# MyNiuuu/MOFA-Video

Hardware: AMD Instinct MI355X
Metric: denoised frames/sec, 25f 576x1024 SVD+MOFA, 25 steps (higher is better)
Workload: dtype f16; 1 GPU; MOFA-Video-Traj, 25-frame 576x1024, 25 denoise steps + temporal VAE decode (chunk 8), single trajectory hint, SVD-XT UNet + MOFA-Adapter, CFG 1->3, seeded random weights in the reference checkpoint layout; num_frames=25, height=576, width=1024, num_inference_steps=25, decode_chunk_size=8, parallelism=1 GPU, graph_steps=False, output_finite=True

## Files before the change

include/mofa_hip.h:

```cpp
#ifndef MOFA_HIP_H
#define MOFA_HIP_H

#include <stdint.h>

#ifdef __cplusplus
extern "C" {
#endif

typedef void* mofa_stream_t;

#define MOFA_OK 0
#define MOFA_EINVAL (-22)
#define MOFA_ELAUNCH (-5)

int mofa_version(void);

enum { MOFA_MODE_PLAIN = 0, MOFA_MODE_CONV3X3 = 1, MOFA_MODE_CONVT3 = 2 };
enum { MOFA_ACT_NONE = 0, MOFA_ACT_SILU = 1, MOFA_ACT_GEGLU_PAIR = 2, MOFA_ACT_RELU = 3,
       MOFA_ACT_GELU = 4  };

typedef struct mofa_igemm_args {
    const void* x;
    const void* w;
    const float* bias;
    const float* rowvec;
    const void* r1;
    const void* r2;
    void* out;
    int32_t M, N, Cin;
    int32_t ldx, ldo, ldr1, ldr2;
    int32_t mode;
    int32_t Hin, Win, Hout, Wout, stride, up, ksize;
    int32_t T, HW;
    int32_t rv_div, rv_mul, rv_mod_in, rv_mod_out;
    int32_t act;
    float s_acc, s1, s2;
    int32_t dil;
    int32_t pad;
    int32_t tile;
    void* workspace;
    int64_t workspace_bytes;
    float* stats;
} mofa_igemm_args;
enum { MOFA_PAD_SAME = 0, MOFA_PAD_TRAILING = 1 };
enum { MOFA_TILE_AUTO = 0, MOFA_TILE_128X128 = 2, MOFA_TILE_192X128 = 4, MOFA_TILE_256X256 = 5, MOFA_TILE_256X320 = 6 };

int mofa_igemm_f16(const mofa_igemm_args* a, mofa_stream_t stream);
int mofa_igemm_stats_ok(const mofa_igemm_args* a);
typedef struct mofa_igemm_plan_t {
    int32_t rc;
    int32_t tile, kind;
    int32_t tiles_m, tiles_n, grid, threads, lds_bytes;
    int32_t split;
    int32_t full_tiles, rem_tiles;
    int32_t stats;
    int32_t launches;
    int32_t reserved[4];
} mofa_igemm_plan_t;
int mofa_igemm_plan(const mofa_igemm_args* a, int n_cu, mofa_igemm_plan_t* out);

int mofa_attn_spatial_f16(const void* q, const void* k, const void* v, void* out,
                          int nframes, int heads, int head_dim, int S, int ldq, int ldk, int ldv, int ldo, float scale,
                          mofa_stream_t stream);
int mofa_attn_spatial_qb_f16(const void* q, const void* k, const void* v, void* out,
                             int nframes, int heads, int head_dim, int S, int ldq, int ldk, int ldv, int ldo, float scale,
                             int query_blocks, mofa_stream_t stream);
int mofa_transpose_v_f16(const void* v, void* vt, int nframes, int ncb, int S, int ldv, mofa_stream_t stream);
int mofa_attn_temporal_f16(const void* q, const void* k, const void* v, void* out,
                           int nclips, int Tq, int T, int HW, int heads, int head_dim, int ld, int ldkv, int ldo,
                           float scale, mofa_stream_t stream);
int mofa_attn_temporal_masked_f16(const void* q, const void* k, const void* v, void* out,
                                  int nclips, int Tq, int T, int HW, int heads, int head_dim, int ld, int ldkv, int ldo,
                                  float scale, uint32_t key_mask, mofa_stream_t stream);
int mofa_attn_temporal_long_f16(const void* q, const void* k, const void* v, void* out,
                                int nclips, int T, int HW, int heads, int head_dim, int ld, int ldkv, int ldo,
                                float scale, mofa_stream_t stream);
int mofa_attn_temporal_long_masked_f16(const void* q, const void* k, const void* v, void* out,
                                       int nclips, int Tq, int T, int HW, int heads, int head_dim, int ld, int ldkv, int ldo,
                                       float scale, const uint32_t* key_mask, mofa_stream_t stream);
int mofa_attn_temporal_long_local_f16(const void* q, const void* k, const void* v, void* out,
                                      int nclips, int T, int HW, int heads, int head_dim, int ld, int ldkv, int ldo,
                                      float scale, int radius, int anchor, mofa_stream_t stream);
int mofa_attn_temporal_stream_local_f16(const void* q, const void* k, const void* v, void* out,
                                        int nclips, int T, int HW, int heads, int head_dim, int ld, int ldkv, int ldo,
                                        float scale, int radius, int anchor, mofa_stream_t stream);
int mofa_softmax_rows_f16(void* x, int rows, int cols, int ld, mofa_stream_t stream);

int mofa_gn_nparts(int HW, int C);
int mofa_gn_partial_f16(const void* x, float* part, int nframes, int HW, int C, int ldx, mofa_stream_t stream);
int mofa_gn_partial_from_stats(const float* stats, float* part, int nframes, int HW, int C, mofa_stream_t stream);
int mofa_gn_finalize(const float* part, const float* gamma, const float* beta, float* scale, float* shift,
                     int nframes, int HW, int C, int frames_per_stat, float eps, mofa_stream_t stream);
int mofa_gn_reduce(const float* part, double* sums, int nframes, int HW, int C, int frames_per_stat, mofa_stream_t stream);
int mofa_gn_finalize_sums(const double* sums, const float* gamma, const float* beta, float* scale, float* shift,
                          int nframes, int C, int frames_per_stat, double count_per_group, float eps,
                          mofa_stream_t stream);
int mofa_gn_apply_f16(const void* x, const float* part, const float* gamma, const float* beta, void* y,
                      int nframes, int HW, int C, int ldx, int ldy, int frames_per_stat, float eps, int silu,
                      mofa_stream_t stream);
int mofa_gn_apply_gathered_f16(const void* x, const float* part_all, int nentries, double count_per_group,
                               const float* gamma, const float* beta, void* y, int nframes, int HW, int C,
                               int ldx, int ldy, float eps, int silu, mofa_stream_t stream);
int mofa_affine_act_f16(const void* x, const float* scale, const float* shift, void* y,
                        int nframes, int HW, int C, int ldx, int ldy, int silu, mofa_stream_t stream);
int mofa_layernorm_f16(const void* x, const float* gamma, const float* beta, void* y, int M, int C,
                       int ldx, int ldy, float eps, const float* rowvec, int rv_div, int rv_mod,
                       mofa_stream_t stream);

typedef struct mofa_ff320_args {
    const void* x;
    const float* pos;
    const void* w1p;
    const float* b1;
    const void* w2p;
    const float* b2;
    const void* r2;
    void* out;
    void* out_ln;
    const float* ln_gamma;
    const float* ln_beta;
    int32_t M, ldx, ldo, ldr2, ldoln, HW, T;
    float eps, s_acc, s1, s2, ln_eps;
    int32_t reserved[4];
} mofa_ff320_args;
int mofa_ff320_f16(const mofa_ff320_args* a, mofa_stream_t stream);

typedef struct mofa_lin320_args {
    const void* x;
    const void* wp;
    const float* bias;
    const float* rowvec;
    const void* r1;
    void* out;
    int32_t M, N, ldx, ldo, ldr1, norm;
    int32_t rv_div, rv_mul, rv_mod_in, rv_mod_out;
    float eps, s_acc, s1;
    int32_t reserved[3];
} mofa_lin320_args;
int mofa_lin320_f16(const mofa_lin320_args* a, mofa_stream_t stream);

int mofa_axpby_f32(const float* x, float* y, int64_t n, float a, float b, mofa_stream_t stream);
int mofa_resize_nearest_f32(const float* x, float* y, int n, int H, int W, int h, int w, mofa_stream_t stream);
int mofa_mask_blend_f16(const void* a, const void* b, const float* w, void* out, int M, int C, int HW, int lda,
                        int ldb, int ldo, mofa_stream_t stream);
int mofa_matting_blend_f16(const void* warped, const void* matting, const void* logit, void* out, float* mask_out,
                           int M, int C, int ldw, int ldm, int ldl, int ldo, mofa_stream_t stream);
int mofa_subsample_tokens_f16(const void* x, void* y, int n, int H, int W, int s, int C, int ldx, int ldy,
                              mofa_stream_t stream);
int mofa_axpby_f16(const void* x, void* y, int M, int C, int ldx, int ldy, float a, float b, mofa_stream_t stream);
int mofa_axpby_out_f16(const void* x, const void* y, void* out, int M, int C, int ldx, int ldy, int ldo, float a, float b,
                       mofa_stream_t stream);
int mofa_geglu_f16(const void* x, void* out, int M, int Ch, int ldx, int ldo, mofa_stream_t stream);
int mofa_copy2d_f16(const void* src, void* dst, int M, int C, int lds, int ldd, mofa_stream_t stream);
int mofa_silu_f32(const float* x, float* y, int n, mofa_stream_t stream);
int mofa_cast_f32_to_f16(const float* x, void* y, int64_t n, mofa_stream_t stream);
int mofa_cast_f16_to_f32(const void* x, float* y, int64_t n, mofa_stream_t stream);
int mofa_nchw_f32_to_nhwc_f16(const float* x, void* y, int n, int C, int HW, int ldo, float scale,
                              mofa_stream_t stream);
int mofa_nhwc_f16_to_nchw_f32(const void* x, float* y, int n, int C, int HW, int ldx, mofa_stream_t stream);
int mofa_timestep_embedding(const float* t, float* out, int n, int dim, mofa_stream_t stream);

int64_t mofa_softsplat_ws_bytes(int nflows, int H, int W);
int mofa_softsplat_avg_f16(const void* feat, const float* flow, void* out, void* ws,
                           int nflows, int H, int W, int C, int ldf, int ldo, mofa_stream_t stream);
int mofa_softsplat_scatter_f32(const float* in, const float* flow, float* out_sum, int N, int C, int H, int W,
                               mofa_stream_t stream);
int mofa_softsplat_weight_f32(const float* in, const float* metric, float* out, int N, int C, int H, int W, int mode,
                              mofa_stream_t stream);
int mofa_softsplat_normalize_f32(const float* summed, float* out, int N, int C, int H, int W, int eps_mode, mofa_stream_t stream);
typedef struct mofa_softsplat_grad_args {
    const float* grad;
    const float* flow;
    const float* in;
    const float* metric;
    const float* inv;
    const float* glast;
    float* grad_in;
    float* grad_flow;
    float* grad_metric;
    float* partial;
    int32_t N, C, H, W, prep, slices;
    int32_t reserved[4];
} mofa_softsplat_grad_args;
int mofa_softsplat_norm_f32(const float* flow, float* norm, void* ws, int N, int H, int W, mofa_stream_t stream);
int mofa_softsplat_grad_prologue_f32(const float* grad, const float* out, const float* norm, float* inv, float* glast,
                                     int N, int C, int H, int W, int eps_mode, mofa_stream_t stream);
int mofa_softsplat_grad_f32(const mofa_softsplat_grad_args* a, mofa_stream_t stream);
typedef struct mofa_softsplat_gather_args {
    const float* in;
    const float* flow;
    const float* metric;
    float* out;
    float* norm;
    void* ws;
    int32_t N, C, H, W, prep, normalize, eps_mode, slices;
    int32_t reserved[4];
} mofa_softsplat_gather_args;
int mofa_softsplat_gather_f32(const mofa_softsplat_gather_args* a, mofa_stream_t stream);
int mofa_flow_downscale_f32(const float* flow, float* out, int n, int H, int W, int s, mofa_stream_t stream);

int mofa_prepare_model_input(const float* latents, const float* image_latents, void* out,
                             int T, int HW, int ldo, float sigma, mofa_stream_t stream);
int mofa_cfg_euler_step(float* latents, const void* noise_pred, int T, int HW, int ldn,
                        float sigma, float sigma_next, float gmin, float gmax, mofa_stream_t stream);
#define MOFA_STEP_SCALARS 8
int mofa_prepare_model_input_dev(const float* latents, const float* image_latents, void* out,
                                 int T, int HW, int ldo, const float* step_scalars, mofa_stream_t stream);
int mofa_cfg_euler_step_dev(float* latents, const void* noise_pred, int T, int HW, int ldn,
                            const float* step_scalars, float gmin, float gmax, mofa_stream_t stream);
int mofa_step_select(const float* table, int* counter, float* cur, int nsteps, mofa_stream_t stream);


// ... 38 lines not shown
```

mofa_video_amd/blocks.py:

```python
import math

import torch

from . import lib as L
from . import ops
from .weights import (f32, interleave_geglu, pack_conv3d_t3, pack_conv3x3, pack_ff320, pack_lin320, pack_linear, pad_rows)

BIG = 1 << 30
LOCAL_STREAM_ABOVE = 128


class Sub:

    def __init__(self, sd, prefix="", device="cuda"):
        self.sd, self.prefix, self.device = sd, prefix, device

    def sub(self, name):
        return Sub(self.sd, f"{self.prefix}{name}.", self.device)

    def has(self, name):
        return f"{self.prefix}{name}" in self.sd

    def get(self, name):
        return self.sd[f"{self.prefix}{name}"].detach()

    def dev(self, t):
        return t.to(self.device)


class Ctx:

    def __init__(self, B, T):
        self.B, self.T = B, T
        self.N = B * T
        self.temb_act = None
        self.temb_all = None
        self.ctx16 = None
        self.cache = {}
        self.time_context_hw_major = True
        self.par = None
        self.ctx16_all = None
        self.half = 0
        self.local = None
        self.halves = None


def make_ctx(net, timestep, encoder_hidden_states, added_time_ids, B, T, base=None, half=None, par=None, local=None):
    c = base if base is not None else Ctx(B, T)
    ts = torch.as_tensor(timestep, dtype=torch.float32, device=net.device).reshape(-1)
    ts = ts.expand(B).contiguous() if ts.numel() == 1 else ts.contiguous()
    ids = added_time_ids.to(net.device, torch.float32)
    if half is not None:
        ids = ids[half:half + B]
    c.temb_act = net.time(ts, ids.contiguous())
    c.temb_all = net.temb_batch.run(c.temb_act)
    if c.ctx16 is None:
        e = encoder_hidden_states.to(net.device, torch.float32)
        e = e.reshape(e.shape[0], -1).contiguous()
        if half is not None:
            c.ctx16_all = ops.cast_f32_to_f16(e)
            c.ctx16 = c.ctx16_all[half:half + B].contiguous()
            c.half = half
        else:
            c.ctx16 = ops.cast_f32_to_f16(e)
    if local is not None and par is not None:
        raise ValueError("local temporal attention of frame-sharded clips: the gathered-key path has no per-query mask")
    c.par, c.local = par, local
    return c


class Linear:
    def __init__(self, s, pad_n=False):
        w = s.get("weight")
        w = w.reshape(w.shape[0], -1)
        self.n_real = w.shape[0]
        b = s.get("bias") if s.has("bias") else None
        if pad_n:
            w = pad_rows(w)
            b = pad_rows(b) if b is not None else None
        self.w = s.dev(pack_linear(w))
        self.b = s.dev(f32(b)) if b is not None else None

    def __call__(self, x, **kw):
        return ops.igemm(x, self.w, self.b, **kw)


class Conv3x3:
    def __init__(self, s, stride=1, up=1, pad_n=False, pad=L.PAD_SAME):
        w, b = s.get("weight"), s.get("bias")
        self.n_real = w.shape[0]
        if pad_n:
            w, b = pad_rows(w), pad_rows(b)
        self.w = s.dev(pack_conv3x3(w))
        self.b = s.dev(f32(b))
        self.stride, self.up, self.pad = stride, up, pad

    def __call__(self, x, H, W, **kw):
        return ops.igemm(x, self.w, self.b, geom=ops.conv3x3_geom(H, W, self.stride, self.up, pad=self.pad), **kw)


class ConvT3:
    def __init__(self, s, pad_n=False):
        w, b = s.get("weight"), s.get("bias")
        if pad_n:
            w, b = pad_rows(w), pad_rows(b)
        self.w = s.dev(pack_conv3d_t3(w))
        self.b = s.dev(f32(b))

    def __call__(self, x, T, HW, **kw):
        return ops.igemm(x, self.w, self.b, geom=ops.convt3_geom(T, HW), **kw)


class GroupNorm:
    def __init__(self, s, eps):
        self.g, self.b, self.eps = s.dev(f32(s.get("weight"))), s.dev(f32(s.get("bias"))), eps

    def __call__(self, x, nframes, HW, frames_per_stat=1, silu=False):
        return ops.group_norm(x, self.g, self.b, nframes, HW, self.eps, frames_per_stat, silu)


class LayerNorm:
    def __init__(self, s, eps=1e-5):
        self.g, self.b, self.eps = s.dev(f32(s.get("weight"))), s.dev(f32(s.get("bias"))), eps

    def __call__(self, x, **kw):
        return ops.layer_norm(x, self.g, self.b, self.eps, **kw)


class GegluFF:

    def __init__(self, s, norm=None, norm_eps=1e-5):
        w, b = interleave_geglu(s.get("net.0.proj.weight"), s.get("net.0.proj.bias"))
        self.w1, self.b1 = s.dev(pack_linear(w)), s.dev(f32(b))
        self.out = Linear(s.sub("net.2"))
        self.pk = None
        if norm is not None and tuple(s.get("net.0.proj.weight").shape) == (2560, 320) and tuple(s.get("net.2.weight").shape) == (320, 1280):
            w1p, b1f, w2p = pack_ff320(s.get("net.0.proj.weight"), s.get("net.0.proj.bias"), s.get("net.2.weight"),
                                       norm.get("weight"), norm.get("bias"))
            self.pk = (s.dev(w1p), s.dev(b1f), s.dev(w2p), norm_eps)

    def __call__(self, x, **epilogue):
        h = ops.igemm(x, self.w1, self.b1, act=L.ACT_GEGLU_PAIR)
        return self.out(h, **epilogue)

    @property
    def can_fuse(self):
        return self.pk is not None and ops.FF_FUSED

    def fused(self, x, **kw):
        w1p, b1f, w2p, eps = self.pk
        return ops.ff320(x, w1p, b1f, w2p, self.out.b, eps=eps, **kw)


def drive(gen):
    try:
        while True:
            next(gen)
    except StopIteration as stop:
        return stop.value


def run_lockstep(gens, enter):
    vals, live = [None] * len(gens), list(range(len(gens)))
    while live:
        for i in list(live):
            with enter[i]():
                try:
                    next(gens[i])
                except StopIteration as stop:
                    vals[i] = stop.value
                    live.remove(i)
    return vals


def _sigmoid(v):
    return 1.0 / (1.0 + math.exp(-float(v)))


class TembBatch:
    _active = None

    def __init__(self):
        self.items, self.total, self.w, self.b = [], 0, None, None

    def __enter__(self):
        self._prev, TembBatch._active = TembBatch._active, self
        return self

    def __exit__(self, *exc):
        TembBatch._active = self._prev
        if exc[0] is None and self.items:
            mult = 1
            for lin in self.items:
                mult = mult * lin.n_real // math.gcd(mult, lin.n_real)
            pad = (-self.total) % mult
            ws, bs = [lin.w for lin in self.items], [lin.b for lin in self.items]
            if pad:
                ws.append(ws[0].new_zeros((pad, ws[0].shape[1])))
                bs.append(bs[0].new_zeros((pad,)))
            self.w, self.b = torch.cat(ws, 0).contiguous(), torch.cat(bs, 0).contiguous()
            for lin in self.items:
                lin.w = lin.b = None
        return False

    def add(self, lin):
        assert lin.w.shape[0] == lin.n_real and lin.n_real % 64 == 0 and lin.b is not None
        off = self.total
        self.items.append(lin)
        self.total += lin.n_real
        return off

    def run(self, temb_act):
        return ops.cast_f16_to_f32(ops.igemm(temb_act, self.w, self.b)) if self.w is not None else None


class SpatioTemporalResBlock:

    def __init__(self, s, eps, temporal_eps=None, switch=False):
        sp, tp = s.sub("spatial_res_block"), s.sub("temporal_res_block")
        self.norm1, self.norm2 = GroupNorm(sp.sub("norm1"), eps), GroupNorm(sp.sub("norm2"), eps)
        self.conv1, self.conv2 = Conv3x3(sp.sub("conv1")), Conv3x3(sp.sub("conv2"))
        self.temb = Linear(sp.sub("time_emb_proj")) if sp.has("time_emb_proj.weight") else None
        tb = TembBatch._active
        self.temb_off = tb.add(self.temb) if (tb is not None and self.temb is not None) else None
        self.shortcut = Linear(sp.sub("conv_shortcut")) if sp.has("conv_shortcut.weight") else None
        te = temporal_eps if temporal_eps is not None else eps
        self.tnorm1, self.tnorm2 = GroupNorm(tp.sub("norm1"), te), GroupNorm(tp.sub("norm2"), te)
        self.tconv1, self.tconv2 = ConvT3(tp.sub("conv1")), ConvT3(tp.sub("conv2"))
        self.ttemb = Linear(tp.sub("time_emb_proj")) if tp.has("time_emb_proj.weight") else None
        self.ttemb_off = tb.add(self.ttemb) if (tb is not None and self.ttemb is not None) else None
        alpha = _sigmoid(s.get("time_mixer.mix_factor").reshape(-1)[0])
        self.alpha = (1.0 - alpha) if switch else alpha

    def __call__(self, x, c, H, W, out_stats=False, out=None):
        HW, N, T = H * W, c.N, c.T

        def tvec(lin, off):
            if off is not None and c.temb_all is not None:
                return dict(rowvec=c.temb_all[:, off:off + lin.n_real], rv=(T * HW, c.temb_all.shape[1] // lin.n_real, 1, BIG))
            return dict(rowvec=ops.cast_f16_to_f32(lin(c.temb_act)), rv=(T * HW, 1, 1, BIG))
        h = self.norm1(x, N, HW, silu=True)
        if self.temb is not None:
            h = self.conv1(h, H, W, stats=True, **tvec(self.temb, self.temb_off))
        else:
            h = self.conv1(h, H, W, stats=True)
        h = self.norm2(h, N, HW, silu=True)
        xs = self.shortcut(x) if self.shortcut is not None else x
        par = c.par
        xs = self.conv2(h, H, W, r1=xs, s1=1.0, stats=par is None)
        if par is None:
# ... 301 lines not shown
```

mofa_video_amd/csrc/igemm.hip:

```cpp
#include "igemm_common.h"


__device__ __forceinline__ void wait_vmcnt_le(int t) {
    if (t >= 48) wait_vmcnt<48>();
    else if (t >= 32) wait_vmcnt<32>();
    else if (t >= 24) wait_vmcnt<24>();
    else if (t >= 16) wait_vmcnt<16>();
    else if (t >= 8) wait_vmcnt<8>();
    else if (t >= 4) wait_vmcnt<4>();
    else wait_vmcnt<0>();
}

#define EPI_SLAB_BYTES 8192
__device__ __forceinline__ int slab_off(int row, int chunk) { return row * 256 + ((chunk ^ (row & 15)) << 4); }

struct PassLoads {
    f16x8 t1, t2;
    f32x4 rv0, rv1;
};

template <int EPI>
__device__ __forceinline__ void load_bias(const mofa_igemm_args& a, int ncol0, int lane, f32x4 (&b)[4]) {
    constexpr bool GEGLU = (EPI & EPI_GEGLU) != 0;
    const f32x4 z = {0, 0, 0, 0};
// ... 241 lines not shown
        for (int q = 0; q < WI; ++q) glds16(wsrc[q] + (size_t)ksw * BKS, sb + SXB + (wave * WI + q) * 1024);
        ++ksw;
        if (++ikc == kpt) { ikc = 0; ++itap; }
    };

    const int fsw = (l31 >> 1) & 7;
    const int xrow = (wm * MI * 32 + l31) * RB;
    const int wrow = SXB + (wn * NJ * 32 + l31) * RB;

    f32x4 bias[4];
    setup(walk.start + walk.local);
    {
        int lane_b = lane;
        asm volatile("" : "+v"(lane_b));
        load_bias<EPI>(a, n0 + wn * NJ * 32, lane_b, bias);
    }
    issue(0);
    int par = 0;
    int allow = 0;
    bool first = true;
    for (;;) {
        const int m0c = m0, n0c = n0;
        f32x16 acc[MI][NJ];
#pragma unroll
        for (int i = 0; i < MI; ++i)
#pragma unroll
            for (int j = 0; j < NJ; ++j)
#pragma unroll
                for (int r = 0; r < 16; ++r) acc[i][j][r] = 0.0f;
        auto compute = [&](int cur) {
            const char* sb = smem + cur * STB;
#pragma unroll
            for (int kk = 0; kk < BKS / 16; ++kk) {
                const int slot = ((kk * 2 + lh) ^ fsw) * 16;
                f16x8 xf[MI], wf[NJ];
#pragma unroll
                for (int i = 0; i < MI; ++i) xf[i] = *(const f16x8*)(sb + xrow + i * 32 * RB + slot);
#pragma unroll
                for (int j = 0; j < NJ; ++j) wf[j] = *(const f16x8*)(sb + wrow + j * 32 * RB + slot);
#pragma unroll
                for (int i = 0; i < MI; ++i)
#pragma unroll
                    for (int j = 0; j < NJ; ++j)
                        acc[i][j] = __builtin_amdgcn_mfma_f32_32x32x16_f16(wf[j], xf[i], acc[i][j], 0, 0, 0);
            }
        };
        auto compute_and_issue = [&](int cur, int nxt) {
            if (ikc == 0) {
#pragma unroll
                for (int q = 0; q < XI; ++q) xs[q] = x_src(a, geo[q], itap);
            }
            const char* sb = smem + cur * STB;
            char* nb = smem + nxt * STB;
            constexpr int OPS = XI + WI, NG = BKS / 16;
            constexpr int SPREAD = 4;
#pragma unroll
            for (int kk = 0; kk < NG; ++kk) {
#pragma unroll
                for (int o = (kk * OPS / SPREAD < OPS ? kk * OPS / SPREAD : OPS);
                     o < ((kk + 1) * OPS / SPREAD < OPS ? (kk + 1) * OPS / SPREAD : OPS); ++o) {
                    if (o < XI) {
                        const f16* sp = xs[o] ? xs[o] + ikc * BKS + xoff[o] : (const f16*)g_zero_page;
                        glds16(sp, nb + (wave * XI + o) * 1024);
                    } else {
                        glds16(wsrc[o - XI] + (size_t)ksw * BKS, nb + SXB + (wave * WI + (o - XI)) * 1024);
                    }
                }
                const int slot = ((kk * 2 + lh) ^ fsw) * 16;
                f16x8 xf[MI], wf[NJ];
#pragma unroll
                for (int i = 0; i < MI; ++i) xf[i] = *(const f16x8*)(sb + xrow + i * 32 * RB + slot);
#pragma unroll
                for (int j = 0; j < NJ; ++j) wf[j] = *(const f16x8*)(sb + wrow + j * 32 * RB + slot);
#pragma unroll
                for (int i = 0; i < MI; ++i)
#pragma unroll
                    for (int j = 0; j < NJ; ++j)
                        acc[i][j] = __builtin_amdgcn_mfma_f32_32x32x16_f16(wf[j], xf[i], acc[i][j], 0, 0, 0);
            }
            ++ksw;
            if (++ikc == kpt) { ikc = 0; ++itap; }
        };
        for (int ks = 0; ks < nk - 1; ++ks) {
            if (ks == 0) wait_vmcnt_le(allow); else wait_vmcnt<0>();
            __builtin_amdgcn_s_barrier();
            const int cur = (par + ks) & 1;
            compute_and_issue(cur, cur ^ 1);
        }
        const int last = (par + nk - 1) & 1;
        if (nk == 1) wait_vmcnt_le(allow); else wait_vmcnt<0>();
        __builtin_amdgcn_s_barrier();
        bias_touch<EPI>(bias);
        walk.local += walk.stride;
        const bool has_next = walk.local < walk.count;
        if (has_next) {
            setup(walk.start + walk.local);
            issue(last ^ 1);
        } else {
#pragma unroll
            for (int q = 0; q < XI + WI; ++q)
                glds16((const f16*)g_zero_page, smem + (last ^ 1) * STB + (wave * (XI + WI) + q) * 1024);
        }
        asm volatile("" ::: "memory");
        compute(last);
        wait_lds();
        __builtin_amdgcn_s_barrier();
        char* slab = smem + last * STB + wave * EPI_SLAB_BYTES;
        int lane_e = lane;
        asm volatile("" : "+v"(lane_e));
        if (wide) igemm_epilogue<MI, EPI, true>(a, acc, m0c + wm * MI * 32, n0c + wn * NJ * 32, lane_e, slab, bias);
        else igemm_epilogue<MI, EPI, false>(a, acc, m0c + wm * MI * 32, n0c + wn * NJ * 32, lane_e, slab, bias);
        first = false;
        if (!has_next) break;
        {
            int lane_b = lane;
            asm volatile("" : "+v"(lane_b));
            load_bias<EPI>(a, n0 + wn * NJ * 32, lane_b, bias);
        }
        allow = (wide && m0c + TBM <= a.M && n0c + TBN <= a.N) ? epi_ops + (a.bias ? (GEGLU ? 4 : 2) : 0) : 0;
        par = last ^ 1;
    }
    wait_vmcnt<0>();
}

extern "C" int mofa_igemm_f16(const mofa_igemm_args* a, mofa_stream_t stream) {
    int rc = igemm_check_args(a);
    if (rc != MOFA_OK) return rc;
#define IGEMM_KINDS(WM, WN, MI)                                                                                        \
    {igemm_f16_kernel<WM, WN, MI, 0>, igemm_f16_kernel<WM, WN, MI, 1>, igemm_f16_kernel<WM, WN, MI, 2>,                \
     igemm_f16_kernel<WM, WN, MI, 3>, igemm_f16_kernel<WM, WN, MI, 4>, igemm_f16_kernel<WM, WN, MI, 5>,                \
     igemm_f16_kernel<WM, WN, MI, 6>, igemm_f16_kernel<WM, WN, MI, 7>, igemm_f16_kernel<WM, WN, MI, 8>}
    static const igemm_kern_t k128[9] = IGEMM_KINDS(2, 2, 2), k192[9] = IGEMM_KINDS(2, 2, 3);
    static LaunchSetup setup;
    const int n_cu = setup.cus([](int) {
        return mofa_lds_optin(k128, igemm_tile(MOFA_TILE_128X128).lds) == MOFA_OK &&
                       mofa_lds_optin(k192, igemm_tile(MOFA_TILE_192X128).lds) == MOFA_OK && igemm8_init() == MOFA_OK &&
                       igemm320_init() == MOFA_OK
                   ? MOFA_OK
                   : MOFA_ELAUNCH;
    });
    if (n_cu == 0) return MOFA_ELAUNCH;
    const IgemmPlan plan = igemm_plan_checked(a, n_cu);
    if (plan.rc != MOFA_OK) return plan.rc;
    if (plan.tile == MOFA_TILE_256X320) return igemm320_launch(a, plan, (hipStream_t)stream);
    if (plan.tile == MOFA_TILE_256X256) return igemm8_launch(a, plan, (hipStream_t)stream);
    hipLaunchKernelGGL((plan.tile == MOFA_TILE_128X128 ? k128 : k192)[plan.kind], dim3(plan.grid), dim3(plan.threads), plan.lds_bytes,
                       (hipStream_t)stream, *a, plan.tiles_n, plan.full_tiles);
    MOFA_CHECK_LAUNCH();
    return MOFA_OK;
}

extern "C" int mofa_igemm_stats_ok(const mofa_igemm_args* a) { return igemm320_stats_ok(a) ? 1 : 0; }

extern "C" int mofa_igemm_plan(const mofa_igemm_args* a, int n_cu, mofa_igemm_plan_t* out) {
    if (!a || !out || n_cu <= 0) return MOFA_EINVAL;
    *out = igemm_plan(a, n_cu);
    return MOFA_OK;
}
```

mofa_video_amd/csrc/igemm320.hip:

```cpp
#include "igemm_common.h"
#include "igemm_pipe.h"

namespace {

constexpr int WN3 = 2, MI3 = 2;
constexpr int TBM3 = 256;
constexpr int RBH = 64;
constexpr int XPL = TBM3 * RBH;
constexpr int NJ3 = 5;
constexpr int TBN3 = WN3 * NJ3 * 32;
constexpr int PLANE = (TBM3 + TBN3) * RBH;
constexpr int SLOT = 2 * PLANE;
constexpr int BIAS0 = 2 * SLOT;
constexpr int LDS_BYTES3 = BIAS0 + 8 * 2 * 768;
constexpr int LOOKAHEAD3 = 4 + NJ3;

struct ScratchRows { __device__ __forceinline__ int operator()(int r) const { return (r >> 3) * 8192 + (r & 7) * 128; } };

__device__ __forceinline__ int slot_swz(int q) { return q ^ ((q & 1) << 1); }

struct Cursor3 {
    int local;
    int ikc, ksw, ky, kx;
    int gx0, gx1;
    unsigned xo0, xo1;
    int phase;
    int kend;
    unsigned wo0;
};

template <int EPI, bool SPLIT = false, bool STATS = false>
__global__ __launch_bounds__(512, 2) void igemm320_f16_kernel(const mofa_igemm_args a, const int tilesN, const int ntiles,
                                                              const Aux aux) {
    constexpr bool R1 = (EPI & EPI_R1) != 0, R2 = (EPI & EPI_R2) != 0, RV = (EPI & EPI_RV) != 0, GEGLU = (EPI & EPI_GEGLU) != 0;
    extern __shared__ __attribute__((aligned(16))) char smem[];
    TileWalk walk;
    walk.init(ntiles);
    const bool has_item = SPLIT && (int)blockIdx.x < aux.nitems;
    if (walk.local >= walk.count && !has_item) return;
    const int tid = threadIdx.x, lane = tid & 63;
    const int wave = __builtin_amdgcn_readfirstlane(tid >> 6);
    const int grp = wave >> 2;
    const int wm = wave / WN3, wn = wave - wm * WN3;
    const int l31 = lane & 31, lh = lane >> 5;

    const int taps = igemm_taps(a);
    const int kpt = a.Cin / 64, nk = taps * kpt;
    const size_t Ktot = (size_t)taps * a.Cin;

    auto swz_bytes = [&](int l, int p) __attribute__((always_inline)) { return (((l & 3) ^ slot_swz((l >> 4) & 3)) * 16 + p * RBH); };
    const TapGeo tg(a);
    const unsigned wd1 = 128u * (unsigned)(Ktot * 2), wd2 = (unsigned)(256 + 16 * (wave & 3) - 16 * wave) * (unsigned)(Ktot * 2);
    constexpr unsigned W_DEAD = 0x80000000u;
    const BufRsrc rsx = buf_rsrc(aux.xbase, aux.x_bytes), rsw = buf_rsrc(a.w, aux.w_bytes);
    const LdsDma16 bglds16;
    auto item_decode = [&](int phase, int local, int& tile, int& kb, int& ke) __attribute__((always_inline)) {
        tile = walk.start + (phase == 0 ? local : 0); kb = 0; ke = nk;
        if constexpr (SPLIT) {
            const int q = fdiv((int)blockIdx.x, aux.nsplit_d), ks = (int)blockIdx.x - q * aux.nsplit;
            const int kb1 = fdiv(ks * nk, aux.nsplit_d), ke1 = fdiv((ks + 1) * nk, aux.nsplit_d);
            const bool it = phase == 1;
            tile = it ? aux.tile0 + q : tile;
            kb = it ? kb1 : 0;
            ke = it ? ke1 : nk;
        }
    };
    auto next_pos = [&](int& phase, int& local) __attribute__((always_inline)) {
        if (phase == 0) {
            local += walk.stride;
            if (local >= walk.count) phase = has_item ? 1 : 2;
        } else {
            phase = 2;
        }
    };
    auto cur_setup = [&](Cursor3& c, const int p) __attribute__((always_inline)) {
        const bool live = c.phase < 2;
        int tile, kb, ke;
        item_decode(c.phase, c.local, tile, kb, ke);
        const int tm = fdiv(tile, aux.tiles_n), tn = tile - tm * tilesN;
        const int l = lane_now(lane), r_l = l >> 2;
        const int g0 = pack_geo(a, aux, tm * TBM3 + 16 * wave + r_l), g1 = pack_geo(a, aux, tm * TBM3 + 16 * (wave + 8) + r_l);
        c.gx0 = live ? g0 : -1;
        c.gx1 = live ? g1 : -1;
        const unsigned wo = (unsigned)(tn * TBN3 + 16 * wave + r_l) * (unsigned)(Ktot * 2) + swz_bytes(l, p);
        c.wo0 = live ? wo : W_DEAD;
        c.ikc = 0; c.ksw = 0; c.ky = 0; c.kx = 0;
        c.kend = ke;
        if constexpr (SPLIT) {
            int tap = fdiv(kb, aux.kpt_d);
            c.ikc = kb - tap * kpt;
            c.ksw = kb;
            if (a.mode == MOFA_MODE_CONV3X3) { c.ky = fdiv(tap, aux.ks_d); c.kx = tap - c.ky * tg.ks; } else c.ky = tap;
            c.xo0 = tap_src(a, aux, tg, c.gx0, c.ky, c.kx, swz_bytes(l, p));
            c.xo1 = tap_src(a, aux, tg, c.gx1, c.ky, c.kx, swz_bytes(l, p));
        }
    };
    auto issue = [&](Cursor3& c, const int p, const int slot) __attribute__((always_inline)) {
        if (c.ikc == 0) {
            const int l = lane_now(lane);
            c.xo0 = tap_src(a, aux, tg, c.gx0, c.ky, c.kx, swz_bytes(l, p));
            c.xo1 = tap_src(a, aux, tg, c.gx1, c.ky, c.kx, swz_bytes(l, p));
        }
        char* pl = smem + slot + p * PLANE;
        const int wk = c.ksw * 128;
        bglds16(rsx, c.xo0, c.ikc * 128, pl + wave * 1024);
        bglds16(rsx, c.xo1, c.ikc * 128, pl + (wave + 8) * 1024);
        bglds16(rsw, c.wo0, wk, pl + XPL + wave * 1024);
        bglds16(rsw, c.wo0 + wd1, wk, pl + XPL + (wave + 8) * 1024);
        if (grp == p) bglds16(rsw, c.wo0 + wd2, wk, pl + XPL + (16 + (wave & 3)) * 1024);
    };
    auto advance = [&](Cursor3& c, const int p) __attribute__((always_inline)) {
        tap_advance(c, a, kpt, tg.ks);
        if (c.ksw == c.kend) { next_pos(c.phase, c.local); cur_setup(c, p); }
    };

    int xa, wa;
    {
        const int r = lane & 15, c = lane >> 4;
        const int rw = 8 * ((r >> 2) & 1) + 4 * (r >> 3) + (r & 3);
        xa = (wm * MI3 * 32 + r) * RBH + (c ^ slot_swz((r >> 2) & 3)) * 16;
        wa = XPL + (wn * NJ3 * 32 + rw) * RBH + (c ^ slot_swz((rw >> 2) & 3)) * 16;
    }

    const BufRsrc rsb = buf_rsrc(a.bias, a.bias ? (unsigned)a.N * 4u : 0u);
    char* bias_lds = smem + BIAS0 + wave * 1536;
    auto bias_prefetch = [&](int phase_, int local_, int slot) __attribute__((always_inline)) {
        if (phase_ != 0) return;
        int tile_, kb_, ke_;
        item_decode(phase_, local_, tile_, kb_, ke_);
        const int tm_ = fdiv(tile_, aux.tiles_n), tn_ = tile_ - tm_ * tilesN;
        const unsigned n0 = (unsigned)(tn_ * TBN3 + wn * NJ3 * 32 + lane_now(lane));
#pragma unroll
        for (int k = 0; k < 3; ++k)
            __builtin_amdgcn_raw_ptr_buffer_load_lds(rsb, (__attribute__((address_space(3))) void*)(bias_lds + slot * 768 + k * 256), 4,
                                                     (n0 + 64u * k) * 4u, 0, 0, 0);
    };

    Cursor3 ca, cb;
    ca.local = cb.local = walk.local;
    ca.phase = cb.phase = walk.local < walk.count ? 0 : 1;
    cur_setup(ca, 0);
    cur_setup(cb, 1);
    bias_prefetch(walk.local < walk.count ? 0 : 1, walk.local, 0);
    issue(ca, 0, 0); advance(ca, 0);
    issue(cb, 1, 0); advance(cb, 1);
    issue(ca, 0, SLOT); advance(ca, 0);
    wait_vmcnt_only<LOOKAHEAD3>();
    __builtin_amdgcn_s_barrier();

    f32x16 acc[MI3][NJ3];
    f16x8 xf[2 * MI3], wf[2 * NJ3];
    auto phase = [&](auto pc, const int bo, const int bn) __attribute__((always_inline)) {
        constexpr int P = decltype(pc)::v;
#pragma unroll
        for (int i = 0; i < 2 * MI3; ++i) xf[i] = *(const f16x8*)(smem + xa + P * PLANE + i * 16 * RBH);
#pragma unroll
        for (int j = 0; j < 2 * NJ3; ++j) wf[j] = *(const f16x8*)(smem + wa + P * PLANE + j * 16 * RBH);
        __builtin_amdgcn_sched_barrier(0);
        if constexpr (P == 0) { issue(cb, 1, bn); advance(cb, 1); }
        else { issue(ca, 0, bo); advance(ca, 0); }
        wait_vmcnt<LOOKAHEAD3>();
        __builtin_amdgcn_sched_barrier(0);
        __builtin_amdgcn_s_barrier();
        __builtin_amdgcn_sched_barrier(0);
        __builtin_amdgcn_s_setprio(1);
#pragma unroll
        for (int i = 0; i < MI3; ++i)
#pragma unroll
            for (int j = 0; j < NJ3; ++j)
#pragma unroll
                for (int q = 0; q < 4; ++q) {
                    f32x4 c = {acc[i][j][4 * q], acc[i][j][4 * q + 1], acc[i][j][4 * q + 2], acc[i][j][4 * q + 3]};
                    c = __builtin_amdgcn_mfma_f32_16x16x32_f16(wf[2 * j + (q >> 1)], xf[2 * i + (q & 1)], c, 0, 0, 0);
#pragma unroll
                    for (int e = 0; e < 4; ++e) acc[i][j][4 * q + e] = c[e];
                }
        __builtin_amdgcn_s_setprio(0);
        __builtin_amdgcn_sched_barrier(0);
        __builtin_amdgcn_s_barrier();
        __builtin_amdgcn_sched_barrier(0);
    };

    auto to_layout32 = [&](f32x16 (&acc)[MI3][NJ3]) __attribute__((always_inline)) {
#pragma unroll
        for (int i = 0; i < MI3; ++i)
#pragma unroll
            for (int j = 0; j < NJ3; ++j)
#pragma unroll
                for (int v = 0; v < 2; ++v)
#pragma unroll
                    for (int s = 0; s < 4; ++s) {
                        const float lo = acc[i][j][8 * v + s], hi = acc[i][j][8 * v + 4 + s];
                        const auto sw = __builtin_amdgcn_permlane16_swap(__builtin_bit_cast(unsigned, lo), __builtin_bit_cast(unsigned, hi), false, false);
                        const unsigned slo = sw[0], shi = sw[1];
                        acc[i][j][8 * v + s] = __builtin_bit_cast(float, slo);
                        acc[i][j][8 * v + 4 + s] = __builtin_bit_cast(float, shi);
                    }
    };

    auto pin_tuples = [&](f32x16 (&acc)[MI3][NJ3]) __attribute__((always_inline)) {
#pragma unroll
        for (int i = 0; i < MI3; ++i)
#pragma unroll
            for (int j = 0; j < NJ3; ++j) asm volatile("" : "+v"(acc[i][j]));
    };

    const ScratchRows srow;
    auto epilogue_light = [&](auto ac, auto wnc, f32x16 (&acc)[MI3][NJ3], const int mw, const int nw, char* eb) __attribute__((always_inline)) {
        constexpr int J0 = decltype(wnc)::v ? 1 : 0;
        constexpr int JS = decltype(wnc)::v ? 0 : 4;
        const int lane_e = lane_now(lane);
        const int lane = lane_e, l31 = lane & 31, lh = lane >> 5;
        f16* out = (f16*)a.out;
        float saccv = a.s_acc;
        asm volatile("" : "+v"(saccv));
        char* wr = eb + srow(l31);
#pragma unroll
        for (int i = 0; i < MI3; ++i) {
#pragma unroll
            for (int pr = 0; pr < 2; ++pr) {
                const int j0 = J0 + 2 * pr;
#pragma unroll
                for (int jj = 0; jj < 2; ++jj)
#pragma unroll
                    for (int g = 0; g < 4; ++g) {
                        f16x4 o;
#pragma unroll
                        for (int e = 0; e < 4; ++e) o[e] = (f16)act_apply(ac, saccv * acc[i][j0 + jj][4 * g + e]);
                        const int c8 = 8 * jj + 2 * g + lh;
                        *(f16x4*)h16_off(wr, l31, c8) = o;
                    }
#pragma unroll
                for (int p = 0; p < 4; ++p) {
                    const H16Piece r = h16_row<8>(eb, srow, lane, p);
                    const int mr = mw + 32 * i + r.row, n = nw + 32 * j0 + 8 * r.blk;
                    if (mr < a.M && n + 8 <= a.N) *(f16x8*)(out + (size_t)mr * a.ldo + n) = r.v;
                }
            }
            {
#pragma unroll
                for (int g = 0; g < 4; ++g) {
                    f16x4 o;
#pragma unroll
                    for (int e = 0; e < 4; ++e) o[e] = (f16)act_apply(ac, saccv * acc[i][JS][4 * g + e]);
                    const int c8 = 2 * g + lh;
                    *(f16x4*)h16_off(wr, l31, c8) = o;
                }
#pragma unroll
                for (int p = 0; p < 2; ++p) {
                    const H16Piece r = h16_row<4>(eb, srow, lane, p);
                    const int mr = mw + 32 * i + r.row, n = nw + 32 * JS + 8 * r.blk;
                    if (mr < a.M && n + 8 <= a.N) *(f16x8*)(out + (size_t)mr * a.ldo + n) = r.v;
                }
            }
        }
        wait_lds();
    };
    auto epilogue_res16 = [&](auto wnc, auto unit, f32x16 (&acc)[MI3][NJ3], const int mw, const int nw, char* eb) __attribute__((always_inline)) {
        constexpr int J0 = decltype(wnc)::v ? 1 : 0;
        constexpr int JS = decltype(wnc)::v ? 0 : 4;
        constexpr bool UNIT = decltype(unit)::v != 0;
        constexpr int PPI = 10, NP = MI3 * PPI;
        const int lane_e = lane_now(lane);
        const int lane = lane_e, l31 = lane & 31, lh = lane >> 5;
        f16* out = (f16*)a.out;
        const f16* r1 = (const f16*)a.r1;
        const f16* r2 = (const f16*)a.r2;
        float s1v = a.s1, s2v = a.s2, saccv = a.s_acc;
        asm volatile("" : "+v"(s1v), "+v"(s2v), "+v"(saccv));
        auto piece_pos = [&](int st, int& mr, int& n) __attribute__((always_inline)) {
            const int i = st / PPI, q = st % PPI;
            if (q < 8) {
                mr = mw + 32 * i + 8 * (q & 3) + (lane >> 3);
                n = nw + 32 * (J0 + 2 * (q >> 2)) + 8 * (lane & 7);
            } else {
                mr = mw + 32 * i + 16 * (q - 8) + (lane >> 2);
                n = nw + 32 * JS + 8 * (lane & 3);
            }
        };
        constexpr int D = (R1 && R2) ? 2 : 5;
        f16x8 L1[D], L2[D];
        auto piece_loads = [&](int st, int slot) __attribute__((always_inline)) {
            int mr, n;
            piece_pos(st, mr, n);
            mr = mr < a.M ? mr : a.M - 1;
            n = n + 8 <= a.N ? n : 0;
            if (R1) L1[slot] = *(const f16x8*)(r1 + (size_t)mr * a.ldr1 + n);
            if (R2) L2[slot] = *(const f16x8*)(r2 + (size_t)mr * a.ldr2 + n);
        };
#pragma unroll
        for (int st = 0; st < D; ++st) piece_loads(st, st);
        auto finish = [&](int st, f16x8 o) __attribute__((always_inline)) {
            int mr, n;
            piece_pos(st, mr, n);
            if constexpr (UNIT) {
                o = o + L1[st % D];
            } else {
#pragma unroll
                for (int e = 0; e < 8; ++e) {
                    float x = (float)o[e];
                    if (R1) x += s1v * (float)L1[st % D][e];
                    if (R2) x += s2v * (float)L2[st % D][e];
                    o[e] = (f16)x;
                }
            }
            if (mr < a.M && n + 8 <= a.N) *(f16x8*)(out + (size_t)mr * a.ldo + n) = o;
            if (st + D < NP) piece_loads(st + D, st % D);
        };
        char* wr = eb + srow(l31);
#pragma unroll
        for (int i = 0; i < MI3; ++i) {
#pragma unroll
            for (int pr = 0; pr < 2; ++pr) {
                const int j0 = J0 + 2 * pr;
#pragma unroll
                for (int jj = 0; jj < 2; ++jj)
#pragma unroll
                    for (int g = 0; g < 4; ++g) {
                        f16x4 o;
#pragma unroll
                        for (int e = 0; e < 4; ++e) o[e] = (f16)(saccv * acc[i][j0 + jj][4 * g + e]);
                        const int c8 = 8 * jj + 2 * g + lh;
                        *(f16x4*)h16_off(wr, l31, c8) = o;
                    }
#pragma unroll
                for (int p = 0; p < 4; ++p) {
                    const H16Piece r = h16_row<8>(eb, srow, lane, p);
                    finish(i * PPI + pr * 4 + p, r.v);
                }
            }
            {
#pragma unroll
                for (int g = 0; g < 4; ++g) {
                    f16x4 o;
#pragma unroll
                    for (int e = 0; e < 4; ++e) o[e] = (f16)(saccv * acc[i][JS][4 * g + e]);
                    const int c8 = 2 * g + lh;
                    *(f16x4*)h16_off(wr, l31, c8) = o;
                }
#pragma unroll
                for (int p = 0; p < 2; ++p) {
                    const H16Piece r = h16_row<4>(eb, srow, lane, p);
                    finish(i * PPI + 8 + p, r.v);
                }
            }
        }
        wait_lds();
    };
    auto epilogue_stats = [&](auto wnc, f32x16 (&acc)[MI3][NJ3], const int mw, const int nw, char* eb) __attribute__((always_inline)) {
        constexpr int J0 = decltype(wnc)::v ? 1 : 0, JS = decltype(wnc)::v ? 0 : 4;
        constexpr int NP = 20;
        const int lane_e = lane_now(lane);
        const int lane = lane_e, l31 = lane & 31, lh = lane >> 5;
        f16* out = (f16*)a.out;
        const f16* r1 = (const f16*)a.r1;
        float saccv = a.s_acc;
        asm volatile("" : "+v"(saccv));
        auto piece_pos = [&](int st, int& mr, int& n) __attribute__((always_inline)) {
            if (st < 16) {
                mr = mw + 32 * ((st >> 2) & 1) + 8 * (st & 3) + (lane >> 3);
                n = nw + 32 * (J0 + 2 * (st >> 3)) + 8 * (lane & 7);
            } else {
                mr = mw + 32 * ((st - 16) >> 1) + 16 * ((st - 16) & 1) + (lane >> 2);
                n = nw + 32 * JS + 8 * (lane & 3);
            }
        };
        constexpr int D = 5;
        f16x8 L1[D];
        auto piece_loads = [&](int st, int slot) __attribute__((always_inline)) {
            int mr, n;
            piece_pos(st, mr, n);
            mr = mr < a.M ? mr : a.M - 1;
            L1[slot] = *(const f16x8*)(r1 + (size_t)mr * a.ldr1 + n);
        };
        if constexpr (R1) {
#pragma unroll
            for (int st = 0; st < D; ++st) piece_loads(st, st);
        }
        float S[4], Q[4];
        const f16x2 one2 = {(f16)1.0f, (f16)1.0f};
        auto finish = [&](int st, f16x8 o) __attribute__((always_inline)) {
            int mr, n;
            piece_pos(st, mr, n);
            if constexpr (R1) o = o + L1[st % D];
            if (mr < a.M) *(f16x8*)(out + (size_t)mr * a.ldo + n) = o;
#pragma unroll
            for (int k = 0; k < 4; ++k) {
                const f16x2 h = {o[2 * k], o[2 * k + 1]};
                S[k] = __builtin_amdgcn_fdot2(h, one2, S[k], false);
                Q[k] = __builtin_amdgcn_fdot2(h, h, Q[k], false);
            }
            asm volatile("" : "+v"(S[0]), "+v"(S[1]), "+v"(S[2]), "+v"(S[3]), "+v"(Q[0]), "+v"(Q[1]), "+v"(Q[2]), "+v"(Q[3]));
            if constexpr (R1) {
                if (st + D < NP) piece_loads(st + D, st % D);
            }
        };
        auto reduce_store = [&](const int from, const int n0, const bool writer) __attribute__((always_inline)) {
#pragma unroll
            for (int o = from; o < 64; o <<= 1) {
                const int src = (lane ^ o) << 2;
#pragma unroll
                for (int k = 0; k < 4; ++k) {
                    S[k] += __builtin_bit_cast(float, __builtin_amdgcn_ds_bpermute(src, __builtin_bit_cast(int, S[k])));
                    Q[k] += __builtin_bit_cast(float, __builtin_amdgcn_ds_bpermute(src, __builtin_bit_cast(int, Q[k])));
                }
// ... 133 lines not shown
                }
            }
        };
#pragma unroll
        for (int st = 0; st < D; ++st) step_loads(st, L[st]);
        char* wr = eb + srow(l31);
        const int wsw = ((l31 >> 1) & 3) | ((l31 & 1) << 2);
#pragma unroll
        for (int st = 0; st < STEPS; ++st) {
            const int i = st / NJ3, j = st % NJ3;
            StepLoads& l = L[st % D];
#pragma unroll
            for (int g = 0; g < 4; ++g) {
                f32x4 v;
#pragma unroll
                for (int e = 0; e < 4; ++e) v[e] = acc[i][j][4 * g + e];
                *(f32x4*)(wr + (((2 * g + lh) ^ wsw) << 4)) = v;
            }
            const int n = nw + 32 * j + 8 * piece;
#pragma unroll
            for (int p = 0; p < 2; ++p) {
                const int row = 16 * p + rrow;
                const int rsw = ((row >> 1) & 3) | ((row & 1) << 2);
                const f32x4 v0 = *(const f32x4*)(eb + srow(row) + (((2 * piece) ^ rsw) << 4));
                const f32x4 v1 = *(const f32x4*)(eb + srow(row) + (((2 * piece + 1) ^ rsw) << 4));
                f16x8 o;
#pragma unroll
                for (int e = 0; e < 4; ++e) {
                    float x0 = v0[e], x1 = v1[e];
                    if (RVROW) { x0 += l.rv0[p][e]; x1 += l.rv1[p][e]; }
                    x0 *= saccv; x1 *= saccv;
                    if (R1 || R2) { x0 = (float)(f16)x0; x1 = (float)(f16)x1; }
                    if (R1) { x0 += s1v * (float)l.t1[p][e]; x1 += s1v * (float)l.t1[p][4 + e]; }
                    if (R2) { x0 += s2v * (float)l.t2[p][e]; x1 += s2v * (float)l.t2[p][4 + e]; }
                    o[e] = (f16)x0; o[4 + e] = (f16)x1;
                }
                const int m = mw + 32 * i + row;
                if (m < a.M && n + 8 <= a.N) *(f16x8*)(out + (size_t)m * a.ldo + n) = o;
            }
            if (st + D < STEPS) step_loads(st + D, L[st % D]);
        }
        wait_lds();
    };

    auto epilogue_dump = [&](f32x16 (&acc)[MI3][NJ3], float* wst, char* eb) __attribute__((always_inline)) {
        const int lane_e = lane_now(lane);
        const int lane = lane_e, l31 = lane & 31, lh = lane >> 5;
        const int piece = lane & 3, rrow = lane >> 2;
        char* wr = eb + srow(l31);
        const int wsw = ((l31 >> 1) & 3) | ((l31 & 1) << 2);
#pragma unroll
        for (int st = 0; st < MI3 * NJ3; ++st) {
            const int i = st / NJ3, j = st % NJ3;
#pragma unroll
            for (int g = 0; g < 4; ++g) {
                f32x4 v;
#pragma unroll
                for (int e = 0; e < 4; ++e) v[e] = acc[i][j][4 * g + e];
                *(f32x4*)(wr + (((2 * g + lh) ^ wsw) << 4)) = v;
            }
#pragma unroll
            for (int p = 0; p < 2; ++p) {
                const int row = 16 * p + rrow;
                const int rsw = ((row >> 1) & 3) | ((row & 1) << 2);
                const f32x4 v0 = *(const f32x4*)(eb + srow(row) + (((2 * piece) ^ rsw) << 4));
                const f32x4 v1 = *(const f32x4*)(eb + srow(row) + (((2 * piece + 1) ^ rsw) << 4));
                float* d = wst + (size_t)(wm * MI3 * 32 + 32 * i + row) * TBN3 + wn * NJ3 * 32 + 32 * j + 8 * piece;
                *(f32x4*)d = v0;
                *(f32x4*)(d + 4) = v1;
            }
        }
        wait_lds();
    };

    int gt = 0;
    int cph = walk.local < walk.count ? 0 : 1, cl = walk.local, bslot = 0;
    for (; cph < 2; next_pos(cph, cl), bslot ^= 1) {
        int tile, kb, ke;
        item_decode(cph, cl, tile, kb, ke);
        {
            int nph = cph, nl = cl;
            next_pos(nph, nl);
            bias_prefetch(nph, nl, bslot ^ 1);
        }
        const int tm = fdiv(tile, aux.tiles_n), tn = tile - tm * tilesN;
        const int mw = tm * TBM3 + wm * MI3 * 32;
        const int nw = tn * TBN3 + wn * NJ3 * 32;
        int idx_u = -1;
        if constexpr (RV) idx_u = rowvec_uniform_idx<32 * MI3>(a, mw);
        if (SPLIT && cph == 1) {
#pragma unroll
            for (int i = 0; i < MI3; ++i)
#pragma unroll
                for (int j = 0; j < NJ3; ++j)
#pragma unroll
                    for (int r = 0; r < 16; ++r) acc[i][j][r] = 0.0f;
        } else {
            const int lane_e = lane_now(lane);
            const int col_e = 8 * ((lane_e >> 4) & 1) + 4 * (lane_e >> 5);
#pragma unroll
            for (int j = 0; j < NJ3; ++j)
#pragma unroll
                for (int v = 0; v < 2; ++v) {
                    f32x4 b = *(const f32x4*)(bias_lds + bslot * 768 + (32 * j + 16 * v + col_e) * 4);
                    if (RV && idx_u >= 0) {
                        int n = nw + 32 * j + 16 * v + col_e;
                        n = n + 4 <= a.N ? n : 0;
                        b += *(const f32x4*)(a.rowvec + (size_t)idx_u * a.N + n);
                    }
#pragma unroll
                    for (int e = 0; e < 4; ++e) {
                        acc[0][j][8 * v + e] = b[e]; acc[0][j][8 * v + 4 + e] = b[e];
                        acc[1][j][8 * v + e] = b[e]; acc[1][j][8 * v + 4 + e] = b[e];
                    }
                }
        }
        pin_tuples(acc);
        if (grp == 1) __builtin_amdgcn_s_barrier();
        for (int kt = kb; kt < ke; ++kt, ++gt) {
            const int bo = (gt & 1) * SLOT, bn = SLOT - bo;
            phase(IC<0>{}, bo, bn);
            phase(IC<1>{}, bo, bn);
            const int d = (gt & 1) ? -SLOT : SLOT;
            xa += d;
            wa += d;
        }
        if (grp == 0) __builtin_amdgcn_s_barrier();
        pin_tuples(acc);
        to_layout32(acc);
        pin_tuples(acc);

        char* eb = smem + ((gt - 1) & 1) * SLOT + PLANE + wave * 1024;
        if (SPLIT && cph == 1) {
            epilogue_dump(acc, aux.ws + (size_t)blockIdx.x * (TBM3 * TBN3), eb);
        } else if constexpr (STATS) {
            if (wn == 0) epilogue_stats(IC<0>{}, acc, mw, nw, eb);
            else epilogue_stats(IC<1>{}, acc, mw, nw, eb);
        } else if constexpr (GEGLU) {
            if (a.s_acc == 1.0f) epilogue_geglu(IC<1>{}, acc, mw, nw, eb);
            else epilogue_geglu(IC<0>{}, acc, mw, nw, eb);
        } else if constexpr (R1 || R2) {
            if (RV && idx_u < 0) {
                epilogue_rows(IC<0>{}, acc, mw, nw, eb);
            } else {
                const bool unit = R1 && !R2 && a.s1 == 1.0f;
                if (wn == 0) {
                    if (unit) epilogue_res16(IC<0>{}, IC<1>{}, acc, mw, nw, eb);
                    else epilogue_res16(IC<0>{}, IC<0>{}, acc, mw, nw, eb);
                } else {
                    if (unit) epilogue_res16(IC<1>{}, IC<1>{}, acc, mw, nw, eb);
                    else epilogue_res16(IC<1>{}, IC<0>{}, acc, mw, nw, eb);
                }
            }
        } else if (RV && idx_u < 0) {
            epilogue_rows(IC<0>{}, acc, mw, nw, eb);
        } else if (wn == 0) {
            if (RV || a.act == MOFA_ACT_NONE) epilogue_light(IC<MOFA_ACT_NONE>{}, IC<0>{}, acc, mw, nw, eb);
            else if (a.act == MOFA_ACT_SILU) epilogue_light(IC<MOFA_ACT_SILU>{}, IC<0>{}, acc, mw, nw, eb);
            else if (a.act == MOFA_ACT_RELU) epilogue_light(IC<MOFA_ACT_RELU>{}, IC<0>{}, acc, mw, nw, eb);
            else epilogue_light(IC<MOFA_ACT_GELU>{}, IC<0>{}, acc, mw, nw, eb);
        } else {
            if (RV || a.act == MOFA_ACT_NONE) epilogue_light(IC<MOFA_ACT_NONE>{}, IC<1>{}, acc, mw, nw, eb);
            else if (a.act == MOFA_ACT_SILU) epilogue_light(IC<MOFA_ACT_SILU>{}, IC<1>{}, acc, mw, nw, eb);
            else if (a.act == MOFA_ACT_RELU) epilogue_light(IC<MOFA_ACT_RELU>{}, IC<1>{}, acc, mw, nw, eb);
            else epilogue_light(IC<MOFA_ACT_GELU>{}, IC<1>{}, acc, mw, nw, eb);
        }
    }
    wait_vmcnt_only<0>();
}

typedef void (*igemm320_kern_t)(const mofa_igemm_args, const int, const int, const Aux);

__global__ __launch_bounds__(256) void igemm320_fixup_kernel(const mofa_igemm_args a, const float* __restrict__ ws, const int tile0,
                                                             const int nsplit, const int tilesN, const int R) {
    constexpr int PPR = TBN3 / 8, PPT = TBM3 * PPR;
    const long long total = (long long)R * PPT;
    for (long long idx = (long long)blockIdx.x * 256 + threadIdx.x; idx < total; idx += (long long)gridDim.x * 256) {
        const int r = (int)(idx / PPT), rem = (int)(idx - (long long)r * PPT);
        const int rr = rem / PPR, pc = rem - rr * PPR;
        const int tile = tile0 + r, tm = tile / tilesN, tn = tile - tm * tilesN;
        const int m = tm * TBM3 + rr, n = tn * TBN3 + pc * 8;
        if (m >= a.M || n + 8 > a.N) continue;
        float v[8];
#pragma unroll
        for (int e = 0; e < 8; ++e) v[e] = 0.f;
        for (int sl = 0; sl < nsplit; ++sl) {
            const float* q = ws + ((size_t)(r * nsplit + sl) * TBM3 + rr) * TBN3 + pc * 8;
            const f32x4 p0 = *(const f32x4*)q, p1 = *(const f32x4*)(q + 4);
#pragma unroll
            for (int e = 0; e < 4; ++e) { v[e] += p0[e]; v[4 + e] += p1[e]; }
        }
        if (a.bias) {
#pragma unroll
            for (int e = 0; e < 8; ++e) v[e] += a.bias[n + e];
        }
        if (a.rowvec) {
            const int idx_rv = ((m / a.rv_div) * a.rv_mul + (m % a.rv_mod_in)) % a.rv_mod_out;
            const float* q = a.rowvec + (size_t)idx_rv * a.N + n;
#pragma unroll
            for (int e = 0; e < 8; ++e) v[e] += q[e];
        }
#pragma unroll
        for (int e = 0; e < 8; ++e) v[e] *= a.s_acc;
        if (a.r1 || a.r2) {
#pragma unroll
            for (int e = 0; e < 8; ++e) v[e] = (float)(f16)v[e];
        }
        if (a.r1) {
            const f16x8 t = *(const f16x8*)((const f16*)a.r1 + (size_t)m * a.ldr1 + n);
#pragma unroll
            for (int e = 0; e < 8; ++e) v[e] += a.s1 * (float)t[e];
        }
        if (a.r2) {
            const f16x8 t = *(const f16x8*)((const f16*)a.r2 + (size_t)m * a.ldr2 + n);
#pragma unroll
            for (int e = 0; e < 8; ++e) v[e] += a.s2 * (float)t[e];
        }
        f16x8 o;
#pragma unroll
        for (int e = 0; e < 8; ++e) {
            float x = v[e];
            if (a.act == MOFA_ACT_SILU) x = silu_f(x);
            else if (a.act == MOFA_ACT_RELU) x = fmaxf(x, 0.0f);
            else if (a.act == MOFA_ACT_GELU) x = gelu_erf_f(x);
            o[e] = (f16)x;
        }
        *(f16x8*)((f16*)a.out + (size_t)m * a.ldo + n) = o;
    }
}

__global__ __launch_bounds__(192) void igemm320_tile_stats_kernel(const f16* __restrict__ out, const int ldo, float* __restrict__ stats,
                                                                  const int M, const int N, const int tile0, const int tilesN) {
    const int tile = tile0 + (int)(blockIdx.x >> 2), tm = tile / tilesN, tn = tile - tm * tilesN;
    const int m0 = tm * TBM3 + 64 * (int)(blockIdx.x & 3), n = tn * TBN3 + 2 * (int)threadIdx.x;
    if (m0 >= M || (int)threadIdx.x >= TBN3 / 2 || n + 2 > N) return;
    const f16x2 one2 = {(f16)1.0f, (f16)1.0f};
    float sm = 0.f, q = 0.f;
    const f16* p = out + (size_t)m0 * ldo + n;
#pragma unroll 8
    for (int r = 0; r < 64; ++r) {
        const f16x2 h = *(const f16x2*)(p + (size_t)r * ldo);
        sm = __builtin_amdgcn_fdot2(h, one2, sm, false);
        q = __builtin_amdgcn_fdot2(h, h, q, false);
    }
    float* sp = stats + (size_t)(m0 >> 6) * N + n;
    sp[0] = sm;
    sp[1] = q;
}

}

static const igemm320_kern_t k_igemm320[9] = {igemm320_f16_kernel<0>, igemm320_f16_kernel<1>, igemm320_f16_kernel<2>,
                                               igemm320_f16_kernel<3>, igemm320_f16_kernel<4>, igemm320_f16_kernel<5>,
                                               igemm320_f16_kernel<6>, nullptr, igemm320_f16_kernel<8>};
static const igemm320_kern_t k_igemm320_split[7] = {
    igemm320_f16_kernel<0, true>, igemm320_f16_kernel<1, true>, igemm320_f16_kernel<2, true>, igemm320_f16_kernel<3, true>,
    igemm320_f16_kernel<4, true>, igemm320_f16_kernel<5, true>, igemm320_f16_kernel<6, true>};

static const igemm320_kern_t k_igemm320_stats[7] = {igemm320_f16_kernel<0, false, true>, igemm320_f16_kernel<1, false, true>, nullptr,
                                                     nullptr, igemm320_f16_kernel<4, false, true>, igemm320_f16_kernel<5, false, true>, nullptr};
static const igemm320_kern_t k_igemm320_split_stats[7] = {igemm320_f16_kernel<0, true, true>, igemm320_f16_kernel<1, true, true>, nullptr,
                                                           nullptr, igemm320_f16_kernel<4, true, true>, igemm320_f16_kernel<5, true, true>, nullptr};

int igemm320_init() {
    return mofa_lds_optin(k_igemm320, LDS_BYTES3) == MOFA_OK && mofa_lds_optin(k_igemm320_split, LDS_BYTES3) == MOFA_OK &&
                   mofa_lds_optin(k_igemm320_stats, LDS_BYTES3) == MOFA_OK && mofa_lds_optin(k_igemm320_split_stats, LDS_BYTES3) == MOFA_OK
               ? MOFA_OK
               : MOFA_ELAUNCH;
}

static_assert(TBM3 == 256 && TBN3 == 320 && LDS_BYTES3 == 159744, "igemm_plan.h's MOFA_TILE_256X320 row");
int igemm320_launch(const mofa_igemm_args* a, const IgemmPlan& plan, hipStream_t stream) {
    const int kind = plan.kind, S = plan.split, R = plan.rem_tiles, tilesN = plan.tiles_n;
    Aux aux = igemm_pipe_aux(a, igemm_taps(*a), tilesN);
    igemm320_kern_t kern = a->stats ? k_igemm320_stats[kind] : k_igemm320[kind];
    if (S > 1) {
        kern = a->stats ? k_igemm320_split_stats[kind] : k_igemm320_split[kind];
        aux.nsplit = S, aux.nsplit_d = fastdiv_make(S);
        aux.tile0 = plan.full_tiles, aux.nitems = R * S, aux.ws = (float*)a->workspace;
    }
    hipLaunchKernelGGL(kern, dim3(plan.grid), dim3(plan.threads), plan.lds_bytes, stream, *a, tilesN, plan.full_tiles, aux);
    MOFA_CHECK_LAUNCH();
    if (S == 1) return MOFA_OK;
    const long long pieces = (long long)R * TBM3 * (TBN3 / 8);
    hipLaunchKernelGGL(igemm320_fixup_kernel, dim3((int)((pieces + 255) / 256)), dim3(256), 0, stream, *a,
                       (const float*)a->workspace, plan.full_tiles, S, tilesN, R);
    MOFA_CHECK_LAUNCH();
    if (a->stats) {
        hipLaunchKernelGGL(igemm320_tile_stats_kernel, dim3(R * 4), dim3(192), 0, stream, (const f16*)a->out, a->ldo, a->stats, a->M,
                           a->N, plan.full_tiles, tilesN);
        MOFA_CHECK_LAUNCH();
    }
    return MOFA_OK;
}
```

mofa_video_amd/csrc/igemm8.hip:

```cpp
#include "igemm_common.h"
#include "igemm_pipe.h"

namespace {

constexpr int WM = 2, WN = 4, MI = 4, NJ = 2;
constexpr int TBM = WM * MI * 32, TBN = WN * NJ * 32;
constexpr int BKS = 64, RB = 128;
constexpr int SXB = TBM * RB, STB = SXB + TBN * RB;
constexpr int SCRATCH0 = 2 * STB, SCRATCH_WAVE = 4096;
constexpr int LDS_BYTES = SCRATCH0 + 8 * SCRATCH_WAVE;
constexpr int LOOKAHEAD_OPS = 8;

struct Cursor {
    int local;
    int ikc, ksw, ky, kx;
    int gx0, gx1;
    unsigned xo0, xo1;
    unsigned wo0, wo1, wo2, wo3;
};

template <int EPI, int VAR = 0>
__global__ __launch_bounds__(512, 2) void igemm8_f16_kernel(const mofa_igemm_args a, const int tilesN, const int ntiles,
                                                            const Aux aux) {
    constexpr bool GEGLU = (EPI & EPI_GEGLU) != 0, R1 = (EPI & EPI_R1) != 0, R2 = (EPI & EPI_R2) != 0,
                   RV = (EPI & EPI_RV) != 0;
    extern __shared__ __attribute__((aligned(16))) char smem[];
    TileWalk walk;
    walk.init(ntiles);
    if (walk.local >= walk.count) return;
    const int tid = threadIdx.x, lane = tid & 63;
    const int wave = __builtin_amdgcn_readfirstlane(tid >> 6);
    const int grp = wave >> 2;
    const int wm = wave / WN, wn = wave - wm * WN;
    const int l31 = lane & 31, lh = lane >> 5;

    const int taps = igemm_taps(a);
    const int kpt = a.Cin / BKS, nk = taps * kpt;
    const size_t Ktot = (size_t)taps * a.Cin;

    auto swz_bytes = [&](int l, int q) __attribute__((always_inline)) { return (((l & 7) ^ (4 * q + (l >> 4))) * 16); };
    auto x_row = [&](int h, int q, int hr0) __attribute__((always_inline)) { const int hr = hr0 + 8 * q; return (hr >> 6) * 128 + h * 64 + (hr & 63); };
    auto w_row = [&](int h, int q, int hr0) __attribute__((always_inline)) { const int hr = hr0 + 8 * q; return (hr >> 5) * 64 + h * 32 + (hr & 31); };
    const TapGeo tg(a);
    const BufRsrc rsx = buf_rsrc(aux.xbase, aux.x_bytes), rsw = buf_rsrc(a.w, aux.w_bytes);
    const LdsDma16 bglds16;
    auto cur_setup = [&](Cursor& c, const int h, const bool with_w) __attribute__((always_inline)) {
        const bool live = c.local < walk.count;
        const int tile = walk.start + (live ? c.local : 0);
        const int tm = fdiv(tile, aux.tiles_n), tn = tile - tm * tilesN;
        const int l = lane_now(lane), hr_l = 16 * wave + (l >> 3);
        const int g0 = pack_geo(a, aux, tm * TBM + x_row(h, 0, hr_l)), g1 = pack_geo(a, aux, tm * TBM + x_row(h, 1, hr_l));
        c.gx0 = live ? g0 : -1;
        c.gx1 = live ? g1 : -1;
        if (with_w) {
            auto w_off = [&](int hq) __attribute__((always_inline)) {
                int n = tn * TBN + w_row(hq >> 1, hq & 1, hr_l);
                n = n < a.N ? n : a.N - 1;
                const unsigned o = (unsigned)n * (unsigned)(Ktot * 2) + swz_bytes(l, hq & 1);
                return live ? o : XO_INVALID;
            };
            c.wo0 = w_off(0); c.wo1 = w_off(1); c.wo2 = w_off(2); c.wo3 = w_off(3);
        }
        c.ikc = 0; c.ksw = 0; c.ky = 0; c.kx = 0;
    };
    auto issue_x = [&](Cursor& c, const int h, const int bo) __attribute__((always_inline)) {
        if (c.ikc == 0) {
            const int l = lane_now(lane);
            c.xo0 = tap_src(a, aux, tg, c.gx0, c.ky, c.kx, swz_bytes(l, 0));
            c.xo1 = tap_src(a, aux, tg, c.gx1, c.ky, c.kx, swz_bytes(l, 1));
        }
        bglds16(rsx, c.xo0, c.ikc * (BKS * 2), smem + bo + x_row(h, 0, 16 * wave) * RB);
        bglds16(rsx, c.xo1, c.ikc * (BKS * 2), smem + bo + x_row(h, 1, 16 * wave) * RB);
    };
    auto issue_w = [&](Cursor& c, const int bo) __attribute__((always_inline)) {
        bglds16(rsw, c.wo0, c.ksw * (BKS * 2), smem + bo + SXB + w_row(0, 0, 16 * wave) * RB);
        bglds16(rsw, c.wo1, c.ksw * (BKS * 2), smem + bo + SXB + w_row(0, 1, 16 * wave) * RB);
        bglds16(rsw, c.wo2, c.ksw * (BKS * 2), smem + bo + SXB + w_row(1, 0, 16 * wave) * RB);
        bglds16(rsw, c.wo3, c.ksw * (BKS * 2), smem + bo + SXB + w_row(1, 1, 16 * wave) * RB);
    };
    auto advance = [&](Cursor& c, const int h, const bool with_w) __attribute__((always_inline)) {
        tap_advance(c, a, kpt, tg.ks);
        if (c.ksw == nk) { c.local += walk.stride; cur_setup(c, h, with_w); }
    };

    int xa[4], wa[4];
    {
        const int fsw = (l31 >> 1) & 7;
#pragma unroll
        for (int kk = 0; kk < 4; ++kk) {
            const int slot = ((kk * 2 + lh) ^ fsw) * 16;
            xa[kk] = (wm * MI * 32 + l31) * RB + slot;
            wa[kk] = SXB + (wn * NJ * 32 + l31) * RB + slot;
        }
    }

    char* scr = smem + SCRATCH0 + wave * SCRATCH_WAVE;
    const BufRsrc rsb = buf_rsrc(a.bias, a.bias ? (unsigned)a.N * 4u : 0u);
    auto bias_prefetch = [&](int nw, int slot = 0) __attribute__((always_inline)) {
        __builtin_amdgcn_raw_ptr_buffer_load_lds(rsb, (__attribute__((address_space(3))) void*)(scr + slot * 256), 4,
                                                 (unsigned)(nw + lane_now(lane)) * 4u, 0, 0, 0);
    };
    constexpr bool BIAS_INIT = GEGLU;

    Cursor ca, cb;
    ca.local = cb.local = walk.local;
    cur_setup(ca, 0, true);
    cur_setup(cb, 1, false);
    if constexpr (BIAS_INIT) {
        const int tile0 = walk.start + walk.local;
        bias_prefetch((tile0 - fdiv(tile0, aux.tiles_n) * tilesN) * TBN + wn * NJ * 32, 0);
    }
    issue_x(ca, 0, 0); issue_w(ca, 0); advance(ca, 0, true);
    issue_x(cb, 1, 0); advance(cb, 1, false);
    issue_x(ca, 0, STB); issue_w(ca, STB); advance(ca, 0, true);
    wait_vmcnt_only<LOOKAHEAD_OPS>();
    __builtin_amdgcn_s_barrier();

    f32x16 acc[MI][NJ];
    f16x8 xf[2][4], wf[2][4];
    unsigned long long tr[13] = {0, 0, 0, 0, 0, 0, 0, 0, 0, 0, 0, 0, 0}, tr_t = 0;
    if (VAR & 64) tr_t = __builtin_readcyclecounter();
    if (VAR & 32) {
#pragma unroll
        for (int kk = 0; kk < 4; ++kk) {
            xf[0][kk] = *(const f16x8*)(smem + xa[kk]);
            xf[1][kk] = *(const f16x8*)(smem + xa[kk] + 32 * RB);
            wf[0][kk] = *(const f16x8*)(smem + wa[kk]);
            wf[1][kk] = *(const f16x8*)(smem + wa[kk] + 32 * RB);
        }
    }
    auto stamp = [&](int k) __attribute__((always_inline)) {
        if (VAR & 64) { const unsigned long long t = __builtin_readcyclecounter(); tr[k] += t - tr_t; tr_t = t; }
    };
    auto phase = [&](auto pc, const int bo, const int bn) __attribute__((always_inline)) {
        constexpr int P = decltype(pc)::v;
        auto reads = [&]() __attribute__((always_inline)) {
            if (VAR & 32) return;
#pragma unroll
            for (int il = 0; il < 2; ++il)
#pragma unroll
                for (int kk = 0; kk < 4; ++kk)
                    xf[il][kk] = *(const f16x8*)(smem + xa[kk] + ((P == 2 ? 2 : 0) + il) * 32 * RB);
            if constexpr (P == 1) {
#pragma unroll
                for (int j = 0; j < 2; ++j)
#pragma unroll
                    for (int kk = 0; kk < 4; ++kk) wf[j][kk] = *(const f16x8*)(smem + wa[kk] + j * 32 * RB);
            }
        };
        auto issues = [&]() __attribute__((always_inline)) {
            if (VAR & 16) return;
            if constexpr (P == 1) issue_x(cb, 1, bn);
            if constexpr (P == 2) { issue_x(ca, 0, bo); issue_w(ca, bo); }
        };
        if (VAR & 4) { issues(); __builtin_amdgcn_sched_barrier(0); reads(); }
        else { reads(); __builtin_amdgcn_sched_barrier(0); issues(); }
        if constexpr (P == 1) advance(cb, 1, false);
        if constexpr (P == 2) advance(ca, 0, true);
        if (!(VAR & 8)) wait_vmcnt<LOOKAHEAD_OPS>(); else wait_lds();
        __builtin_amdgcn_sched_barrier(0);
        __builtin_amdgcn_s_barrier();
        __builtin_amdgcn_sched_barrier(0);
        stamp(3 * (P - 1));
        if (!(VAR & 2)) __builtin_amdgcn_s_setprio(1);
#pragma unroll
        for (int kk = 0; kk < 4; ++kk)
#pragma unroll
            for (int il = 0; il < 2; ++il)
#pragma unroll
                for (int j = 0; j < 2; ++j) {
                    constexpr int I0 = (P == 2) ? 2 : 0;
                    acc[I0 + il][j] = __builtin_amdgcn_mfma_f32_32x32x16_f16(wf[j][kk], xf[il][kk], acc[I0 + il][j], 0, 0, 0);
                }
        if (!(VAR & 2)) __builtin_amdgcn_s_setprio(0);
        stamp(3 * (P - 1) + 1);
        __builtin_amdgcn_sched_barrier(0);
        __builtin_amdgcn_s_barrier();
        __builtin_amdgcn_sched_barrier(0);
        stamp(3 * (P - 1) + 2);
    };

    auto epilogue_light = [&](auto ac, auto un, f32x16 (&acc)[MI][NJ], const int mw, const int nw, const int idx_u) __attribute__((always_inline)) {
        constexpr bool UNI = decltype(un)::v != 0;
        constexpr bool SACC1 = GEGLU && UNI;
        const int lane_e = RV ? lane_now(lane) : lane;
        const int lane = lane_e, l31 = lane & 31, lh = lane >> 5;
        f16* out = (f16*)a.out;
        float saccv = a.s_acc;
        asm volatile("" : "+v"(saccv));
        f32x4 bv[NJ][4];
        if (!BIAS_INIT && (!RV || UNI)) {
#pragma unroll
            for (int j = 0; j < NJ; ++j)
#pragma unroll
                for (int g = 0; g < 4; ++g) bv[j][g] = *(const f32x4*)(scr + (32 * j + 8 * g + 4 * lh) * 4);
        }
        const int nout = GEGLU ? a.N / 2 : a.N;
        int rv_div = a.rv_div, rv_mod_in = a.rv_mod_in, rv_mod_out = a.rv_mod_out;
        asm volatile("" : "+s"(rv_div), "+s"(rv_mod_in), "+s"(rv_mod_out));
        f32x4 rv[NJ][4];
        auto rv_load = [&](int i, f32x4 (&rv)[NJ][4]) __attribute__((always_inline)) {
            int m = mw + 32 * i + l31;
            m = m < a.M ? m : a.M - 1;
            const int idx = UNI ? idx_u : ((m / rv_div) * a.rv_mul + (m % rv_mod_in)) % rv_mod_out;
            const float* rvp = a.rowvec + (size_t)idx * a.N;
#pragma unroll
            for (int j = 0; j < NJ; ++j)
#pragma unroll
                for (int g = 0; g < 4; ++g) {
                    int n = nw + 32 * j + 8 * g + 4 * lh;
                    n = n + 4 <= a.N ? n : 0;
                    rv[j][g] = *(const f32x4*)(rvp + n);
                    if (!UNI && a.bias) rv[j][g] += *(const f32x4*)(a.bias + n);
                }
        };
        if (RV) rv_load(0, rv);
        if (RV && UNI) {
#pragma unroll
            for (int j = 0; j < NJ; ++j)
#pragma unroll
                for (int g = 0; g < 4; ++g) bv[j][g] += rv[j][g];
        }
        auto store_pair = [&](f16x4 g0, f16x4 g1, int m, int n0) __attribute__((always_inline)) {
            typedef unsigned u32x2 __attribute__((ext_vector_type(2)));
            typedef unsigned u32x4 __attribute__((ext_vector_type(4)));
            u32x2 a2 = __builtin_bit_cast(u32x2, g0), b2 = __builtin_bit_cast(u32x2, g1);
            const auto rx = __builtin_amdgcn_permlane32_swap(a2[0], b2[0], false, false);
            const auto ry = __builtin_amdgcn_permlane32_swap(a2[1], b2[1], false, false);
            const u32x4 v = {rx[0], ry[0], rx[1], ry[1]};
            const int n = n0 + 8 * lh;
            if (m < a.M && n + 8 <= nout) *(u32x4*)(out + (size_t)m * a.ldo + n) = v;
        };
#pragma unroll
        for (int i = 0; i < MI; ++i) {
            const int m = mw + 32 * i + l31;
            if constexpr (GEGLU) {
                f16x4 o[4];
#pragma unroll
                for (int g = 0; g < 4; ++g)
#pragma unroll
                    for (int e = 0; e < 4; ++e) {
                        const float val = acc[i][g >> 1][4 * (g & 1) + e];
                        const float gate = acc[i][g >> 1][8 + 4 * (g & 1) + e];
                        if constexpr (SACC1) o[g][e] = (f16)(val * (gate * gelu_phi_f(gate)));
                        else o[g][e] = (f16)(saccv * val * gelu_erf_f(saccv * gate));
                    }
                store_pair(o[0], o[1], m, nw / 2);
                store_pair(o[2], o[3], m, nw / 2 + 16);
            } else {
#pragma unroll
                for (int j = 0; j < NJ; ++j)
#pragma unroll
                    for (int g = 0; g < 4; ++g) {
                        f16x4 o;
#pragma unroll
                        for (int e = 0; e < 4; ++e) {
                            const float v = acc[i][j][4 * g + e] + (RV && !UNI ? rv[j][g][e] : bv[j][g][e]);
                            o[e] = (f16)act_apply(ac, saccv * v);
                        }
                        *(f16x4*)(scr + h16_off(l31 * 128, l31, 8 * j + 2 * g + lh)) = o;
                    }
                if (RV && !UNI && i + 1 < MI) rv_load(i + 1, rv);
#pragma unroll
                for (int p = 0; p < 4; ++p) {
                    const H16Piece r = h16_row<4 * NJ>(scr, RowLines128{}, lane, p);
                    const int mr = mw + 32 * i + r.row, n = nw + 8 * r.blk;
                    if (mr < a.M && n + 8 <= nout) *(f16x8*)(out + (size_t)mr * a.ldo + n) = r.v;
                }
            }
        }
    };
    auto epilogue_residual = [&](auto un, f32x16 (&acc)[MI][NJ], const int mw, const int nw, const int idx_u) __attribute__((always_inline)) {
        constexpr bool UNI = decltype(un)::v != 0;
        constexpr int STEPS = MI * NJ;
        constexpr int REGS = (R1 ? 8 : 0) + (R2 ? 8 : 0) + (RV && !UNI ? 16 : 0);
        constexpr int D0 = REGS <= 8 ? 8 : (REGS <= 16 ? 4 : (REGS <= 24 ? 2 : 1));
        constexpr int D = RV && UNI ? (REGS <= 8 ? 4 : 2) : (RV ? 1 : D0);
        const int lane_e = RV ? lane_now(lane) : lane;
        const int lane = lane_e, l31 = lane & 31, lh = lane >> 5;
        f16* out = (f16*)a.out;
        const f16* r1 = (const f16*)a.r1;
        const f16* r2 = (const f16*)a.r2;
        float s1v = a.s1, s2v = a.s2, saccv = a.s_acc;
        asm volatile("" : "+v"(s1v), "+v"(s2v), "+v"(saccv));
        int rv_div = a.rv_div, rv_mod_in = a.rv_mod_in, rv_mod_out = a.rv_mod_out;
        asm volatile("" : "+s"(rv_div), "+s"(rv_mod_in), "+s"(rv_mod_out));
        const int piece = lane & 3;
        struct StepLoads { f16x8 t1[2], t2[2]; f32x4 rv0[2], rv1[2]; };
        StepLoads L[D];
        auto step_loads = [&](int st, StepLoads& l) __attribute__((always_inline)) {
            const int i = st / NJ, j = st % NJ;
            const int n = nw + 32 * j + 8 * piece;
            const int nc = n + 8 <= a.N ? n : 0;
#pragma unroll
            for (int p = 0; p < 2; ++p) {
                int m = mw + 32 * i + 16 * p + (lane >> 2);
                m = m < a.M ? m : a.M - 1;
                if (R1) l.t1[p] = *(const f16x8*)(r1 + (size_t)m * a.ldr1 + nc);
                if (R2) l.t2[p] = *(const f16x8*)(r2 + (size_t)m * a.ldr2 + nc);
                if (RV && !UNI) {
                    const int idx = ((m / rv_div) * a.rv_mul + (m % rv_mod_in)) % rv_mod_out;
                    const float* q = a.rowvec + (size_t)idx * a.N + nc;
                    l.rv0[p] = *(const f32x4*)q;
                    l.rv1[p] = *(const f32x4*)(q + 4);
                }
            }
        };
        f32x4 rvu[NJ][2];
        if (RV && UNI) {
#pragma unroll
            for (int j = 0; j < NJ; ++j) {
                const int n = nw + 32 * j + 8 * piece;
                const float* q = a.rowvec + (size_t)idx_u * a.N + (n + 8 <= a.N ? n : 0);
                rvu[j][0] = *(const f32x4*)q;
                rvu[j][1] = *(const f32x4*)(q + 4);
            }
        }
#pragma unroll
        for (int st = 0; st < D && st < STEPS; ++st) step_loads(st, L[st]);
        f32x4 bv[NJ][2];
#pragma unroll
        for (int j = 0; j < NJ; ++j) {
            bv[j][0] = *(const f32x4*)(scr + (32 * j + 8 * piece) * 4);
            bv[j][1] = *(const f32x4*)(scr + (32 * j + 8 * piece + 4) * 4);
            if (RV && UNI) { bv[j][0] += rvu[j][0]; bv[j][1] += rvu[j][1]; }
        }
#pragma unroll
        for (int st = 0; st < STEPS; ++st) {
            const int i = st / NJ, j = st % NJ;
            StepLoads& l = L[st % D];
#pragma unroll
            for (int g = 0; g < 4; ++g) {
                f32x4 v;
#pragma unroll
                for (int e = 0; e < 4; ++e) v[e] = acc[i][j][4 * g + e];
                *(f32x4*)(scr + f32_off(l31 * 128, l31, 2 * g + lh)) = v;
            }
            const int n = nw + 32 * j + 8 * piece;
#pragma unroll
            for (int p = 0; p < 2; ++p) {
                const int row = 16 * p + (lane >> 2);
                const f32x4 v0 = *(const f32x4*)(scr + f32_off(row * 128, row, 2 * piece));
                const f32x4 v1 = *(const f32x4*)(scr + f32_off(row * 128, row, 2 * piece + 1));
                f16x8 o;
#pragma unroll
                for (int e = 0; e < 4; ++e) {
                    float x0 = v0[e] + bv[j][0][e], x1 = v1[e] + bv[j][1][e];
                    if (RV && !UNI) { x0 += l.rv0[p][e]; x1 += l.rv1[p][e]; }
                    x0 *= saccv; x1 *= saccv;
                    if (R1 || R2) { x0 = (float)(f16)x0; x1 = (float)(f16)x1; }
                    if (R1) { x0 += s1v * (float)l.t1[p][e]; x1 += s1v * (float)l.t1[p][4 + e]; }
                    if (R2) { x0 += s2v * (float)l.t2[p][e]; x1 += s2v * (float)l.t2[p][4 + e]; }
                    o[e] = (f16)x0; o[4 + e] = (f16)x1;
                }
                const int m = mw + 32 * i + row;
                if (m < a.M && n + 8 <= a.N) *(f16x8*)(out + (size_t)m * a.ldo + n) = o;
            }
            if (st + D < STEPS) step_loads(st + D, L[st % D]);
        }
    };

    int gt = 0;
    int bslot = 0;
    for (int cl = walk.local; cl < walk.count; cl += walk.stride, bslot ^= 1) {
        const int tile = walk.start + cl;
        const int tm = fdiv(tile, aux.tiles_n), tn = tile - tm * tilesN;
        if (VAR & 64) { stamp(9); tr[12] += nk; }
        if constexpr (BIAS_INIT) {
            int tn2 = tn;
            if (cl + walk.stride < walk.count) {
                const int tile2 = walk.start + cl + walk.stride;
                tn2 = tile2 - fdiv(tile2, aux.tiles_n) * tilesN;
            }
            bias_prefetch(tn2 * TBN + wn * NJ * 32, bslot ^ 1);
            const int lh_e = lane_now(lane) >> 5;
#pragma unroll
            for (int j = 0; j < NJ; ++j)
#pragma unroll
                for (int g = 0; g < 4; ++g) {
                    const f32x4 b = *(const f32x4*)(scr + bslot * 256 + (32 * j + 8 * g + 4 * lh_e) * 4);
#pragma unroll
                    for (int i = 0; i < MI; ++i)
#pragma unroll
                        for (int e = 0; e < 4; ++e) acc[i][j][4 * g + e] = b[e];
                }
        } else {
#pragma unroll
            for (int i = 0; i < MI; ++i)
#pragma unroll
                for (int j = 0; j < NJ; ++j)
#pragma unroll
                    for (int r = 0; r < 16; ++r) acc[i][j][r] = 0.0f;

            bias_prefetch(tn * TBN + wn * NJ * 32);
        }
        if (!(VAR & 1) && grp == 1) __builtin_amdgcn_s_barrier();
        for (int kt = 0; kt < nk; ++kt, ++gt) {
            const int bo = (gt & 1) * STB, bn = STB - bo;
            phase(IC<1>{}, bo, bn);
            phase(IC<2>{}, bo, bn);
#pragma unroll
            for (int kk = 0; kk < 4; ++kk) { xa[kk] ^= STB; wa[kk] ^= STB; }
        }
        if (!(VAR & 1) && grp == 0) __builtin_amdgcn_s_barrier();
        stamp(6);

        const int mw = tm * TBM + wm * MI * 32;
        const int nw = tn * TBN + wn * NJ * 32;
        int idx_u = -1;
        if constexpr (RV) idx_u = rowvec_uniform_idx<32 * MI>(a, mw);
        if constexpr (R1 || R2) {
            if (RV && idx_u >= 0) epilogue_residual(IC<1>{}, acc, mw, nw, idx_u);
            else epilogue_residual(IC<0>{}, acc, mw, nw, 0);
        } else if constexpr (GEGLU) {
            if (a.s_acc == 1.0f) epilogue_light(IC<MOFA_ACT_NONE>{}, IC<1>{}, acc, mw, nw, 0);
            else epilogue_light(IC<MOFA_ACT_NONE>{}, IC<0>{}, acc, mw, nw, 0);
        } else if constexpr (RV) {
            if (idx_u >= 0) epilogue_light(IC<MOFA_ACT_NONE>{}, IC<1>{}, acc, mw, nw, idx_u);
            else epilogue_light(IC<MOFA_ACT_NONE>{}, IC<0>{}, acc, mw, nw, 0);
        } else {
            if (a.act == MOFA_ACT_NONE) epilogue_light(IC<MOFA_ACT_NONE>{}, IC<0>{}, acc, mw, nw, 0);
            else if (a.act == MOFA_ACT_SILU) epilogue_light(IC<MOFA_ACT_SILU>{}, IC<0>{}, acc, mw, nw, 0);
            else if (a.act == MOFA_ACT_RELU) epilogue_light(IC<MOFA_ACT_RELU>{}, IC<0>{}, acc, mw, nw, 0);
            else epilogue_light(IC<MOFA_ACT_GELU>{}, IC<0>{}, acc, mw, nw, 0);
        }
        if (VAR & 64) { stamp(7); tr[8] += 1; }
    }
    wait_vmcnt_only<0>();
    if ((VAR & 64) && aux.trace && (tid & 255) == 0) {
#pragma unroll
        for (int k = 0; k < 13; ++k) aux.trace[((size_t)blockIdx.x * 2 + grp) * 16 + k] = tr[k];
    }
}

typedef void (*igemm8_kern_t)(const mofa_igemm_args, const int, const int, const Aux);

}

static const igemm8_kern_t k_igemm8[9] = {igemm8_f16_kernel<0>, igemm8_f16_kernel<1>, igemm8_f16_kernel<2>,
                                           igemm8_f16_kernel<3>, igemm8_f16_kernel<4>, igemm8_f16_kernel<5>,
                                           igemm8_f16_kernel<6>, igemm8_f16_kernel<7>, igemm8_f16_kernel<8>};


#ifdef MOFA_PROBE
static int s_probe_var = 0;
static unsigned long long* s_probe_trace = nullptr;
static const int k_probe_vars[] = {1, 2, 4, 8, 16, 32, 48, 64};
static const igemm8_kern_t k_trace_kern[9] = {nullptr, igemm8_f16_kernel<1, 64>, nullptr, nullptr, igemm8_f16_kernel<4, 64>, nullptr, nullptr,
                                               nullptr, igemm8_f16_kernel<8, 64>};
static const igemm8_kern_t k_probe_kern[] = {
    igemm8_f16_kernel<0, 1>, igemm8_f16_kernel<0, 2>, igemm8_f16_kernel<0, 4>, igemm8_f16_kernel<0, 8>,
    igemm8_f16_kernel<0, 16>, igemm8_f16_kernel<0, 32>, igemm8_f16_kernel<0, 48>, igemm8_f16_kernel<0, 64>};
extern "C" int mofa_igemm8_set_probe(int var, void* trace) {
    s_probe_var = var;
    s_probe_trace = (unsigned long long*)trace;
    return 0;
}
#endif

int igemm8_init() {
    if (mofa_lds_optin(k_igemm8, LDS_BYTES) != MOFA_OK) return MOFA_ELAUNCH;
#ifdef MOFA_PROBE
    if (mofa_lds_optin(k_probe_kern, LDS_BYTES) != MOFA_OK || mofa_lds_optin(k_trace_kern, LDS_BYTES) != MOFA_OK) return MOFA_ELAUNCH;
#endif
    return MOFA_OK;
}

int igemm8_launch(const mofa_igemm_args* a, const IgemmPlan& plan, hipStream_t stream) {
    static_assert(TBM == 256 && TBN == 256 && LDS_BYTES == 163840, "igemm_plan.h's MOFA_TILE_256X256 row");
    const int kind = plan.kind;
    Aux aux = igemm_pipe_aux(a, igemm_taps(*a), plan.tiles_n);
    igemm8_kern_t kern = k_igemm8[kind];
#ifdef MOFA_PROBE
    aux.trace = s_probe_trace;
    if (kind == 0 && s_probe_var)
        for (size_t i = 0; i < sizeof(k_probe_vars) / sizeof(int); ++i)
            if (k_probe_vars[i] == s_probe_var) kern = k_probe_kern[i];
    if (s_probe_var == 64 && k_trace_kern[kind]) kern = k_trace_kern[kind];
#endif
    hipLaunchKernelGGL(kern, dim3(plan.grid), dim3(plan.threads), plan.lds_bytes, stream, *a, plan.tiles_n, plan.full_tiles, aux);
    MOFA_CHECK_LAUNCH();
    return MOFA_OK;
}
```

mofa_video_amd/csrc/igemm_pipe.h:

```cpp
#pragma once
#include "igemm_common.h"

namespace {

struct FastDiv { unsigned mul, shr; };
__device__ __forceinline__ int fdiv(int n, const FastDiv d) { return d.mul ? (int)(__umulhi((unsigned)n, d.mul) >> d.shr) : n; }

struct Aux {
    FastDiv tiles_n, hw, wout, t3hw, t3t;
    int ldxb;
    int row_shift;
    const void* xbase;
    unsigned x_bytes, w_bytes;
    unsigned long long* trace;
    FastDiv nsplit_d, kpt_d, ks_d;
    int nsplit, tile0, nitems;
    float* ws;
};

constexpr unsigned XO_INVALID = 0xffffffffu;

template <int V> struct IC { static constexpr int v = V; };

__device__ __forceinline__ int lane_now(int lane) { asm volatile("" : "+v"(lane)); return lane; }

struct TapGeo {
    int ks, dil, org;
    __device__ __forceinline__ TapGeo(const mofa_igemm_args& a)
        : ks(a.ksize > 0 ? a.ksize : 3), dil(a.dil > 0 ? a.dil : 1), org(a.pad == MOFA_PAD_TRAILING ? 0 : (ks >> 1)) {}
};

__device__ __forceinline__ int pack_geo(const mofa_igemm_args& a, const Aux& aux, int m) {
    int g = m;
    if (a.mode == MOFA_MODE_CONV3X3) {
        const int img = fdiv(m, aux.hw), rem = m - img * (a.Hout * a.Wout);
        const int oy = fdiv(rem, aux.wout);
        g = (img << 20) | (oy << 10) | (rem - oy * a.Wout);
    } else if (a.mode == MOFA_MODE_CONVT3) {
        int lo = 1, hi = 1;
        if (a.T > 0) {
            const int fr = fdiv(m, aux.t3hw);
            const int f = fr - fdiv(fr, aux.t3t) * a.T;
            lo = f > 0; hi = f < a.T - 1;
        }
        g = m | (lo << 29) | (hi << 30);
    }
    return m < a.M ? g : -1;
}

__device__ __forceinline__ unsigned tap_src(const mofa_igemm_args& a, const Aux& aux, const TapGeo& t, int g, int ky, int kx, int swzb) {
    int row = g;
    bool ok = g >= 0;
    if (a.mode == MOFA_MODE_CONV3X3) {
        const int vy = ((g >> 10) & 1023) * a.stride + (ky - t.org) * t.dil;
        const int vx = (g & 1023) * a.stride + (kx - t.org) * t.dil;
        ok = ok && vy >= 0 && vx >= 0 && vy < a.Hin * a.up && vx < a.Win * a.up;
        const int iy = (a.up == 2) ? (vy >> 1) : vy, ix = (a.up == 2) ? (vx >> 1) : vx;
        row = ((g >> 20) * a.Hin + iy) * a.Win + ix;
    } else if (a.mode == MOFA_MODE_CONVT3) {
        ok = ok && !(ky == 0 && !((g >> 29) & 1)) && !(ky == 2 && !((g >> 30) & 1));
        row = (g & 0x1fffffff) + (ky - 1) * a.HW + aux.row_shift;
    }
    const unsigned off = (unsigned)row * (unsigned)aux.ldxb + (unsigned)swzb;
    return ok ? off : XO_INVALID;
}

template <class C>
__device__ __forceinline__ void tap_advance(C& c, const mofa_igemm_args& a, const int kpt, const int ks) {
    ++c.ksw;
    if (++c.ikc == kpt) {
        c.ikc = 0;
        if (a.mode == MOFA_MODE_CONV3X3) { if (++c.kx == ks) { c.kx = 0; ++c.ky; } } else ++c.ky;
    }
}

typedef decltype(__builtin_amdgcn_make_buffer_rsrc((void*)nullptr, (short)0, 0, 0)) BufRsrc;
__device__ __forceinline__ BufRsrc buf_rsrc(const void* p, unsigned bytes) {
    return __builtin_amdgcn_make_buffer_rsrc((void*)p, 0, bytes, 0x00020000);
}
struct LdsDma16 {
    __device__ __forceinline__ void operator()(const BufRsrc& rs, unsigned voff, int soff, char* lds_wave_base) const {
        __builtin_amdgcn_raw_ptr_buffer_load_lds(rs, (__attribute__((address_space(3))) void*)lds_wave_base, 16, voff, soff, 0, 0);
    }
};

template <int ACT>
__device__ __forceinline__ float act_apply(IC<ACT>, float v) {
    if constexpr (ACT == MOFA_ACT_SILU) return silu_f(v);
    else if constexpr (ACT == MOFA_ACT_RELU) return fmaxf(v, 0.0f);
    else if constexpr (ACT == MOFA_ACT_GELU) return gelu_erf_f(v);
    else return v;
}

template <int ROWS>
__device__ __forceinline__ int rowvec_uniform_idx(const mofa_igemm_args& a, const int mw) {
    int idx_u = -1;
    if (a.rv_mod_in == 1) {
        int rv_div = a.rv_div;
        asm volatile("" : "+s"(rv_div));
        const int m0 = mw < a.M ? mw : a.M - 1, m1 = mw + ROWS - 1 < a.M ? mw + ROWS - 1 : a.M - 1;
        const int q0 = m0 / rv_div, q1 = m1 / rv_div;
        if (q0 == q1) idx_u = (q0 * a.rv_mul) % a.rv_mod_out;
    }
    return __builtin_amdgcn_readfirstlane(idx_u);
}

struct RowLines128 { __device__ __forceinline__ int operator()(int r) const { return r * 128; } };
template <class B>
__device__ __forceinline__ B h16_off(B rb, int r, int c8) {
    return rb + (((c8 >> 1) ^ ((r >> 1) & 7)) << 4) + (((c8 & 1) ^ (r & 1)) << 3);
}
__device__ __forceinline__ f16x8 h16_row_fix(int r, f16x8 v) {
    f16x8 o = v;
    if (r & 1) o = (f16x8){v[4], v[5], v[6], v[7], v[0], v[1], v[2], v[3]};
    return o;
}
template <class B>
__device__ __forceinline__ B f32_off(B rb, int r, int c) {
    return rb + ((c ^ (((r >> 1) & 3) | ((r & 1) << 2))) << 4);
}

struct H16Piece { int row, blk; f16x8 v; };
template <int CPR, class RowLines>
__device__ __forceinline__ H16Piece h16_row(const char* sb, RowLines rl, int lane, int p) {
    constexpr int SH = CPR == 8 ? 3 : (CPR == 4 ? 2 : 1);
    static_assert(CPR == 1 << SH, "8, 4 or 2 pieces per row");
    const int row = (64 >> SH) * p + (lane >> SH), blk = lane & (CPR - 1);
    const f16x8 v = *(const f16x8*)(sb + rl(row) + ((blk ^ ((row >> 1) & 7)) << 4));
    return H16Piece{row, blk, h16_row_fix(row, v)};
}

}

static inline FastDiv fastdiv_make(int d) {
    FastDiv f = {0, 0};
    if (d > 1) {
        unsigned lg = 0;
        while ((1u << lg) < (unsigned)d) ++lg;
        const unsigned p = 31 + lg;
        f.mul = (unsigned)(((1ull << p) + (unsigned)d - 1) / (unsigned)d);
        f.shr = p - 32;
    }
    return f;
}

static inline Aux igemm_pipe_aux(const mofa_igemm_args* a, int taps, int tilesN) {
    Aux aux;
    aux.tiles_n = fastdiv_make(tilesN);
    aux.hw = fastdiv_make(a->mode == MOFA_MODE_CONV3X3 ? a->Hout * a->Wout : 1);
    aux.wout = fastdiv_make(a->mode == MOFA_MODE_CONV3X3 ? a->Wout : 1);
    aux.t3hw = fastdiv_make(a->mode == MOFA_MODE_CONVT3 ? a->HW : 1);
    aux.t3t = fastdiv_make(a->mode == MOFA_MODE_CONVT3 && a->T > 0 ? a->T : 1);
    const bool halo = a->mode == MOFA_MODE_CONVT3 && a->T == 0;
    aux.ldxb = a->ldx * 2;
    aux.row_shift = halo ? a->HW : 0;
    aux.xbase = (const char*)a->x - (halo ? (size_t)a->HW * a->ldx * 2 : 0);
    aux.x_bytes = (unsigned)(igemm8_rows_in(a) * a->ldx * 2 - (a->ldx - a->Cin) * 2);
    aux.w_bytes = (unsigned)((long long)a->N * taps * a->Cin * 2);
    aux.trace = nullptr;
    aux.nsplit_d = fastdiv_make(1);
    aux.kpt_d = fastdiv_make(a->Cin / 64);
    aux.ks_d = fastdiv_make(a->mode == MOFA_MODE_CONV3X3 ? (a->ksize > 0 ? a->ksize : 3) : 1);
    aux.nsplit = 1;
    aux.tile0 = 0;
    aux.nitems = 0;
    aux.ws = nullptr;
    return aux;
}
```

mofa_video_amd/csrc/igemm_plan.h:

```cpp
#pragma once
#include <stdint.h>
#include "../../include/mofa_hip.h"

typedef mofa_igemm_plan_t IgemmPlan;

struct IgemmTile { int tm, tn, threads, lds, wg_per_cu; };
static inline const IgemmTile& igemm_tile(int id) {
    static const IgemmTile tiles[4] = {
        {128, 128, 256, 2 * 256 * 128, 2},
        {192, 128, 256, 2 * 320 * 128, 2},
        {256, 256, 512, 163840, 1},
        {256, 320, 512, 159744, 1},
    };
    return tiles[id == MOFA_TILE_128X128 ? 0 : id == MOFA_TILE_192X128 ? 1 : id == MOFA_TILE_256X256 ? 2 : 3];
}

static inline int igemm_cdiv(int64_t a, int64_t b) { return (int)((a + b - 1) / b); }

__attribute__((always_inline)) constexpr int igemm_taps(const mofa_igemm_args& a) {
    return (a.mode == MOFA_MODE_CONV3X3) ? (a.ksize > 0 ? a.ksize * a.ksize : 9) : (a.mode == MOFA_MODE_CONVT3 ? 3 : 1);
}

static inline int igemm_grid(long long ntiles, int slots) {
    const int grid = (int)(ntiles < slots ? ((ntiles + 7) / 8) * 8 : (slots / 8) * 8);
    return grid < 8 ? 8 : grid;
}

static inline long long igemm8_rows_in(const mofa_igemm_args* a) {
    if (a->mode == MOFA_MODE_CONV3X3) return a->M / ((long long)a->Hout * a->Wout) * a->Hin * a->Win;
    if (a->mode == MOFA_MODE_CONVT3 && a->T == 0) return (long long)a->M + 2ll * a->HW;
    return a->M;
}

static inline bool igemm_pipe_eligible(const mofa_igemm_args* a, int kind, long long Ktot) {
    const int nout = kind == 8 ? a->N / 2 : a->N;
    if ((a->ldo & 7) || (nout & 7) || (a->N & 7) || (((uintptr_t)a->out) & 15) || (((uintptr_t)a->x) & 15)) return false;
    if (a->r1 && ((a->ldr1 & 7) || (((uintptr_t)a->r1) & 15))) return false;
    if (a->r2 && ((a->ldr2 & 7) || (((uintptr_t)a->r2) & 15))) return false;
    if (a->bias && (((uintptr_t)a->bias) & 15)) return false;
    if ((a->r1 || a->r2 || a->rowvec) && a->act != MOFA_ACT_NONE) return false;
    if (a->rowvec && (((uintptr_t)a->rowvec) & 15)) return false;
    if ((long long)a->N * Ktot * 2 >= (1ll << 32) || (((uintptr_t)a->w) & 15)) return false;
    if (a->mode == MOFA_MODE_CONV3X3) {
        const long long nimg = a->M / ((long long)a->Hout * a->Wout);
        if (a->Hout > 1024 || a->Wout > 1024 || nimg > 2047) return false;
    } else if (a->mode == MOFA_MODE_CONVT3) {
        if (a->M >= (1 << 29)) return false;
    }
    if (igemm8_rows_in(a) * a->ldx * 2 >= (1ll << 32) - 65536) return false;
    return true;
}

static inline bool igemm320_eligible(const mofa_igemm_args* a, int kind, int taps) {
    if (kind == 7 || !igemm_pipe_eligible(a, kind, (long long)taps * a->Cin)) return false;
    return (long long)(a->N + 320) * taps * a->Cin * 2 < 0x7ff00000LL;
}

static inline bool igemm320_stats_ok(const mofa_igemm_args* a) {
    if (!a || !a->x || !a->w || !a->out || a->M <= 0 || a->N <= 0 || a->Cin <= 0 || a->Cin % 64 != 0) return false;
    if (a->act != MOFA_ACT_NONE || a->r2 || (a->r1 && a->s1 != 1.0f)) return false;
    if (a->M % 64 != 0 || a->N % 320 != 0) return false;
    if (a->rowvec && (a->rv_mod_in != 1 || a->rv_div <= 0 || a->rv_div % 64 != 0)) return false;
    if (a->tile != 0 && a->tile != MOFA_TILE_256X320) return false;
    return igemm320_eligible(a, (a->r1 ? 1 : 0) | (a->rowvec ? 4 : 0), igemm_taps(*a));
}

static inline int igemm320_split(long long T, int nk, int n_cu, long long ws_bytes) {
    const long long R = T % n_cu;
    if (ws_bytes <= 0 || R == 0) return 1;
    if (T > n_cu && R * 10 > (long long)n_cu * 6) return 1;
    long long s = n_cu / R;
    if (s > 8) s = 8;
    if (s > nk / 8) s = nk / 8;
    if (s >= 2 && 2.0 * nk * (1.0 - 1.0 / (double)s) < 50.0) s = 1;
    const long long per = (long long)256 * 320 * 4;
    while (s >= 2 && R * s * per > ws_bytes) --s;
    return s >= 2 ? (int)s : 1;
}

static inline int igemm_check_args(const mofa_igemm_args* a) {
    if (!a || !a->x || !a->w || !a->out) return MOFA_EINVAL;
    if (a->M <= 0 || a->N <= 0 || a->Cin <= 0) return MOFA_EINVAL;
    if (a->Cin % 64 != 0 || a->N % 4 != 0) return MOFA_EINVAL;
    if (a->mode < 0 || a->mode > 2 || a->act < 0 || a->act > MOFA_ACT_GELU) return MOFA_EINVAL;
    if (a->mode == MOFA_MODE_CONV3X3) {
        if (a->Hin <= 0 || a->Win <= 0 || a->Hout <= 0 || a->Wout <= 0) return MOFA_EINVAL;
        if ((a->stride != 1 && a->stride != 2) || (a->up != 1 && a->up != 2)) return MOFA_EINVAL;
        if (a->ksize != 0 && a->ksize != 1 && a->ksize != 3 && a->ksize != 5 && a->ksize != 7) return MOFA_EINVAL;
        if (a->dil < 0 || (a->dil > 1 && a->up != 1)) return MOFA_EINVAL;
        if (a->pad != MOFA_PAD_SAME && a->pad != MOFA_PAD_TRAILING) return MOFA_EINVAL;
        if (a->M % (a->Hout * a->Wout) != 0 || a->Hout > 65535 || a->Wout > 65535) return MOFA_EINVAL;
    }
    if (a->mode == MOFA_MODE_CONVT3 && (a->T < 0 || a->HW <= 0 || (a->T > 0 && a->M % (a->T * a->HW) != 0)))
        return MOFA_EINVAL;
    if (a->rowvec && (a->rv_div <= 0 || a->rv_mod_in <= 0 || a->rv_mod_out <= 0)) return MOFA_EINVAL;
    if (a->act == MOFA_ACT_GEGLU_PAIR && (a->N % 64 != 0 || a->r1 || a->r2 || a->rowvec)) return MOFA_EINVAL;
    if (a->ldx % 8 != 0 || a->ldo % 4 != 0) return MOFA_EINVAL;
    if ((a->r1 && a->ldr1 % 4 != 0) || (a->r2 && a->ldr2 % 4 != 0)) return MOFA_EINVAL;
    if (a->tile != 0 && a->tile != MOFA_TILE_128X128 && a->tile != MOFA_TILE_192X128 && a->tile != MOFA_TILE_256X256 &&
        a->tile != MOFA_TILE_256X320)
        return MOFA_EINVAL;
    if (a->stats && !igemm320_stats_ok(a)) return MOFA_EINVAL;
    return MOFA_OK;
}

static inline int igemm_model_tile(const mofa_igemm_args* a, int kind, long long Ktot, int n_cu) {
    static const double rel[2] = {1.00, 0.86};
    static const int ids[2] = {MOFA_TILE_128X128, MOFA_TILE_192X128};
    static const double epi4[9] = {2.0, 3.5, 4.0, 4.0, 3.5, 4.0, 4.5, 4.5, 4.0};
    static const double epi8[9] = {2.2, 5.2, 5.2, 6.0, 5.6, 5.5, 5.5, 6.3, 2.4};
    const double nk = (double)(Ktot / 64);
    int choice = 0;
    double best = 0;
    for (int k = 0; k < 2; ++k) {
        const IgemmTile& c = igemm_tile(ids[k]);
        const long long t = (long long)igemm_cdiv(a->M, c.tm) * igemm_cdiv(a->N, c.tn);
        const long long slots_k = (long long)n_cu * c.wg_per_cu;
        const double cost = (double)((t + slots_k - 1) / slots_k) * c.tm * c.tn * rel[k] * c.wg_per_cu * (1.0 + epi4[kind] / nk);
        if (choice == 0 || cost < best) { best = cost; choice = ids[k]; }
    }
    {
        const long long t = (long long)igemm_cdiv(a->M, 256) * igemm_cdiv(a->N, 256);
        const double cost = (double)((t + n_cu - 1) / n_cu) * 256 * 256 * 0.62 * (1.0 + epi8[kind] / nk);
        if (cost < best) { best = cost; choice = MOFA_TILE_256X256; }
    }
    if (kind != 7) {
        static const double epi320[9] = {3.0, 7.5, 8.5, 9.5, 3.5, 7.9, 9.0, 12.0, 5.0};
        const long long t = (long long)igemm_cdiv(a->M, 256) * igemm_cdiv(a->N, 320);
        const int S = kind == 8 ? 1 : igemm320_split(t, (int)nk, n_cu, a->workspace ? a->workspace_bytes : 0);
        const double rounds = S > 1 ? (double)(t / n_cu) + 1.0 / S + 0.12 : (double)((t + n_cu - 1) / n_cu);
        const int tn320 = igemm_cdiv(a->N, 320);
        const double wide = 1.0 + (tn320 > 6 ? (tn320 - 6 > 12 ? 0.25 : 0.02 * (tn320 - 6)) : 0.0);
        const double cost = rounds * 256 * 320 * 0.58 * wide * (1.0 + epi320[kind] / nk);
        if (cost < best) { best = cost; choice = MOFA_TILE_256X320; }
    }
    return choice;
}

static inline IgemmPlan igemm_plan_checked(const mofa_igemm_args* a, int n_cu) {
    IgemmPlan p = {};
    const IgemmPlan refused = {MOFA_EINVAL};
    n_cu = n_cu >= 8 ? (n_cu / 8) * 8 : 8;
    const int taps = igemm_taps(*a);
    const long long Ktot = (long long)taps * a->Cin;
    const int kind = a->act == MOFA_ACT_GEGLU_PAIR ? 8 : ((a->r1 ? 1 : 0) | (a->r2 ? 2 : 0) | (a->rowvec ? 4 : 0));
    const bool forced = a->tile != 0 || a->stats;
    int choice = a->stats ? MOFA_TILE_256X320 : a->tile != 0 ? a->tile : igemm_model_tile(a, kind, Ktot, n_cu);
    static const int chain[3] = {MOFA_TILE_256X320, MOFA_TILE_256X256, MOFA_TILE_192X128};
    for (int i = 0; i < 2; ++i) {
        if (choice != chain[i]) continue;
        if (i == 0 ? (a->stats || igemm320_eligible(a, kind, taps)) : igemm_pipe_eligible(a, kind, Ktot)) break;
        if (forced) return refused;
        choice = chain[i + 1];
    }
    const IgemmTile& c = igemm_tile(choice);
    const int tilesM = igemm_cdiv(a->M, c.tm), tilesN = igemm_cdiv(a->N, c.tn);
    const long long nt = (long long)tilesM * tilesN;
    if (nt > 0x7fffffffLL) return refused;
    if (a->stats && (((uintptr_t)a->stats) & 15)) return refused;
    const int slots = n_cu * c.wg_per_cu;
    p.tile = choice; p.kind = kind; p.tiles_m = tilesM; p.tiles_n = tilesN; p.threads = c.threads; p.lds_bytes = c.lds;
    p.grid = igemm_grid(nt, slots);
    p.split = 1; p.full_tiles = (int)nt; p.launches = 1;
    p.stats = a->stats ? 1 : 0;
    if (choice == MOFA_TILE_256X320 && kind != 8) {
        const bool ws_ok = a->workspace && (((uintptr_t)a->workspace) & 15) == 0;
        p.split = igemm320_split(nt, (int)(Ktot / 64), n_cu, ws_ok ? a->workspace_bytes : 0);
    }
    if (p.split > 1) {
        p.full_tiles = (int)(nt - nt % n_cu);
        p.rem_tiles = (int)(nt % n_cu);
        p.grid = p.full_tiles > 0 ? (n_cu / 8) * 8 : ((p.rem_tiles * p.split + 7) / 8) * 8;
        p.launches = a->stats ? 3 : 2;
        if (p.grid < p.rem_tiles * p.split) return refused;
    }
    return p;
}

static inline IgemmPlan igemm_plan(const mofa_igemm_args* a, int n_cu) {
    const IgemmPlan refused = {igemm_check_args(a)};
    return refused.rc == MOFA_OK ? igemm_plan_checked(a, n_cu) : refused;
}
```

mofa_video_amd/lib.py:

```python
import ctypes as C
import os

import torch

_HERE = os.path.dirname(os.path.abspath(__file__))
LIB_PATH = os.environ.get("MOFA_HIP_LIB") or os.path.join(_HERE, "libmofa_hip.so")

MODE_PLAIN, MODE_CONV3X3, MODE_CONVT3 = 0, 1, 2
ACT_NONE, ACT_SILU, ACT_GEGLU_PAIR, ACT_RELU, ACT_GELU = 0, 1, 2, 3, 4
PAD_SAME, PAD_TRAILING = 0, 1
SPARSE_ADD, SPARSE_LAST = 0, 1
TILE_AUTO, TILE_128X128, TILE_192X128, TILE_256X256, TILE_256X320 = 0, 2, 4, 5, 6


class IgemmArgs(C.Structure):
    _fields_ = [
        ("x", C.c_void_p), ("w", C.c_void_p), ("bias", C.c_void_p), ("rowvec", C.c_void_p),
        ("r1", C.c_void_p), ("r2", C.c_void_p), ("out", C.c_void_p),
        ("M", C.c_int32), ("N", C.c_int32), ("Cin", C.c_int32),
        ("ldx", C.c_int32), ("ldo", C.c_int32), ("ldr1", C.c_int32), ("ldr2", C.c_int32),
        ("mode", C.c_int32),
        ("Hin", C.c_int32), ("Win", C.c_int32), ("Hout", C.c_int32), ("Wout", C.c_int32),
        ("stride", C.c_int32), ("up", C.c_int32), ("ksize", C.c_int32),
        ("T", C.c_int32), ("HW", C.c_int32),
        ("rv_div", C.c_int32), ("rv_mul", C.c_int32), ("rv_mod_in", C.c_int32), ("rv_mod_out", C.c_int32),
        ("act", C.c_int32),
        ("s_acc", C.c_float), ("s1", C.c_float), ("s2", C.c_float),
        ("dil", C.c_int32), ("pad", C.c_int32), ("tile", C.c_int32),
        ("workspace", C.c_void_p), ("workspace_bytes", C.c_int64),
        ("stats", C.c_void_p),
    ]


class IgemmPlan(C.Structure):
    _fields_ = [(n, C.c_int32) for n in ("rc", "tile", "kind", "tiles_m", "tiles_n", "grid", "threads", "lds_bytes", "split",
                                         "full_tiles", "rem_tiles", "stats", "launches")] + [("reserved", C.c_int32 * 4)]


class Ff320Args(C.Structure):
    _fields_ = [
        ("x", C.c_void_p), ("pos", C.c_void_p), ("w1p", C.c_void_p), ("b1", C.c_void_p), ("w2p", C.c_void_p), ("b2", C.c_void_p),
        ("r2", C.c_void_p), ("out", C.c_void_p), ("out_ln", C.c_void_p), ("ln_gamma", C.c_void_p), ("ln_beta", C.c_void_p),
        ("M", C.c_int32), ("ldx", C.c_int32), ("ldo", C.c_int32), ("ldr2", C.c_int32), ("ldoln", C.c_int32),
        ("HW", C.c_int32), ("T", C.c_int32),
        ("eps", C.c_float), ("s_acc", C.c_float), ("s1", C.c_float), ("s2", C.c_float), ("ln_eps", C.c_float),
        ("reserved", C.c_int32 * 4),
    ]


class Lin320Args(C.Structure):
    _fields_ = [
        ("x", C.c_void_p), ("wp", C.c_void_p), ("bias", C.c_void_p), ("rowvec", C.c_void_p), ("r1", C.c_void_p), ("out", C.c_void_p),
        ("M", C.c_int32), ("N", C.c_int32), ("ldx", C.c_int32), ("ldo", C.c_int32), ("ldr1", C.c_int32), ("norm", C.c_int32),
        ("rv_div", C.c_int32), ("rv_mul", C.c_int32), ("rv_mod_in", C.c_int32), ("rv_mod_out", C.c_int32),
        ("eps", C.c_float), ("s_acc", C.c_float), ("s1", C.c_float),
        ("reserved", C.c_int32 * 3),
    ]


class SoftsplatGradArgs(C.Structure):
    _fields_ = [
        ("grad", C.c_void_p), ("flow", C.c_void_p), ("inp", C.c_void_p), ("metric", C.c_void_p), ("inv", C.c_void_p),
        ("glast", C.c_void_p), ("grad_in", C.c_void_p), ("grad_flow", C.c_void_p), ("grad_metric", C.c_void_p),
        ("partial", C.c_void_p),
        ("N", C.c_int32), ("C", C.c_int32), ("H", C.c_int32), ("W", C.c_int32), ("prep", C.c_int32), ("slices", C.c_int32),
        ("reserved", C.c_int32 * 4),
    ]


class SoftsplatGatherArgs(C.Structure):
    _fields_ = [
        ("inp", C.c_void_p), ("flow", C.c_void_p), ("metric", C.c_void_p), ("out", C.c_void_p), ("norm", C.c_void_p), ("ws", C.c_void_p),
        ("N", C.c_int32), ("C", C.c_int32), ("H", C.c_int32), ("W", C.c_int32), ("prep", C.c_int32), ("normalize", C.c_int32),
        ("eps_mode", C.c_int32), ("slices", C.c_int32),
        ("reserved", C.c_int32 * 4),
    ]


_P, _I, _F, _L = C.c_void_p, C.c_int, C.c_float, C.c_int64

PROTOTYPES = {
    "mofa_version": [],
    "mofa_igemm_f16": [_P, _P],
    "mofa_igemm_stats_ok": [_P],
    "mofa_igemm_plan": [_P, _I, _P],
    "mofa_ff320_f16": [_P, _P],
    "mofa_lin320_f16": [_P, _P],
    "mofa_attn_spatial_f16": [_P, _P, _P, _P, _I, _I, _I, _I, _I, _I, _I, _I, _F, _P],
    "mofa_attn_spatial_qb_f16": [_P, _P, _P, _P, _I, _I, _I, _I, _I, _I, _I, _I, _F, _I, _P],
    "mofa_transpose_v_f16": [_P, _P, _I, _I, _I, _I, _P],
    "mofa_attn_temporal_f16": [_P, _P, _P, _P, _I, _I, _I, _I, _I, _I, _I, _I, _I, _F, _P],
    "mofa_attn_temporal_masked_f16": [_P, _P, _P, _P, _I, _I, _I, _I, _I, _I, _I, _I, _I, _F, C.c_uint32, _P],
    "mofa_attn_temporal_long_f16": [_P, _P, _P, _P, _I, _I, _I, _I, _I, _I, _I, _I, _F, _P],
    "mofa_attn_temporal_long_masked_f16": [_P, _P, _P, _P, _I, _I, _I, _I, _I, _I, _I, _I, _I, _F, _P, _P],
    "mofa_attn_temporal_long_local_f16": [_P, _P, _P, _P, _I, _I, _I, _I, _I, _I, _I, _I, _F, _I, _I, _P],
    "mofa_attn_temporal_stream_local_f16": [_P, _P, _P, _P, _I, _I, _I, _I, _I, _I, _I, _I, _F, _I, _I, _P],
    "mofa_softmax_rows_f16": [_P, _I, _I, _I, _P],
    "mofa_gn_nparts": [_I, _I],
    "mofa_gn_partial_f16": [_P, _P, _I, _I, _I, _I, _P],
    "mofa_gn_partial_from_stats": [_P, _P, _I, _I, _I, _P],
    "mofa_gn_finalize": [_P, _P, _P, _P, _P, _I, _I, _I, _I, _F, _P],
    "mofa_gn_reduce": [_P, _P, _I, _I, _I, _I, _P],
    "mofa_gn_finalize_sums": [_P, _P, _P, _P, _P, _I, _I, _I, C.c_double, _F, _P],
    "mofa_gn_apply_f16": [_P, _P, _P, _P, _P, _I, _I, _I, _I, _I, _I, _F, _I, _P],
    "mofa_gn_apply_gathered_f16": [_P, _P, _I, C.c_double, _P, _P, _P, _I, _I, _I, _I, _I, _F, _I, _P],
    "mofa_affine_act_f16": [_P, _P, _P, _P, _I, _I, _I, _I, _I, _I, _P],
    "mofa_layernorm_f16": [_P, _P, _P, _P, _I, _I, _I, _I, _F, _P, _I, _I, _P],
    "mofa_axpby_f32": [_P, _P, _L, _F, _F, _P],
    "mofa_resize_nearest_f32": [_P, _P, _I, _I, _I, _I, _I, _P],
    "mofa_mask_blend_f16": [_P, _P, _P, _P, _I, _I, _I, _I, _I, _I, _P],
    "mofa_matting_blend_f16": [_P, _P, _P, _P, _P, _I, _I, _I, _I, _I, _I, _P],
    "mofa_subsample_tokens_f16": [_P, _P, _I, _I, _I, _I, _I, _I, _I, _P],
    "mofa_axpby_f16": [_P, _P, _I, _I, _I, _I, _F, _F, _P],
    "mofa_axpby_out_f16": [_P, _P, _P, _I, _I, _I, _I, _I, _F, _F, _P],
    "mofa_geglu_f16": [_P, _P, _I, _I, _I, _I, _P],
    "mofa_copy2d_f16": [_P, _P, _I, _I, _I, _I, _P],
    "mofa_silu_f32": [_P, _P, _I, _P],
    "mofa_cast_f32_to_f16": [_P, _P, _L, _P],
    "mofa_cast_f16_to_f32": [_P, _P, _L, _P],
    "mofa_nchw_f32_to_nhwc_f16": [_P, _P, _I, _I, _I, _I, _F, _P],
    "mofa_nhwc_f16_to_nchw_f32": [_P, _P, _I, _I, _I, _I, _P],
    "mofa_timestep_embedding": [_P, _P, _I, _I, _P],
    "mofa_softsplat_ws_bytes": [_I, _I, _I],
    "mofa_softsplat_avg_f16": [_P, _P, _P, _P, _I, _I, _I, _I, _I, _I, _P],
    "mofa_softsplat_scatter_f32": [_P, _P, _P, _I, _I, _I, _I, _P],
    "mofa_softsplat_weight_f32": [_P, _P, _P, _I, _I, _I, _I, _I, _P],
    "mofa_softsplat_normalize_f32": [_P, _P, _I, _I, _I, _I, _I, _P],
    "mofa_softsplat_norm_f32": [_P, _P, _P, _I, _I, _I, _P],
    "mofa_softsplat_grad_prologue_f32": [_P, _P, _P, _P, _P, _I, _I, _I, _I, _I, _P],
    "mofa_softsplat_grad_f32": [_P, _P],
    "mofa_softsplat_gather_f32": [_P, _P],
    "mofa_flow_downscale_f32": [_P, _P, _I, _I, _I, _I, _P],
    "mofa_prepare_model_input": [_P, _P, _P, _I, _I, _I, _F, _P],
    "mofa_cfg_euler_step": [_P, _P, _I, _I, _I, _F, _F, _F, _F, _P],
    "mofa_prepare_model_input_dev": [_P, _P, _P, _I, _I, _I, _P, _P],
    "mofa_cfg_euler_step_dev": [_P, _P, _I, _I, _I, _P, _F, _F, _P],
    "mofa_step_select": [_P, _P, _P, _I, _P],
    "mofa_pool2d_f16": [_P, _P, _I, _I, _I, _I, _I, _I, _I, _I, _I, _I, _P],
    "mofa_resize_bilinear_ac_f16": [_P, _P, _I, _I, _I, _I, _I, _I, _I, _I, _P],
    "mofa_resize_bilinear_ac_f32": [_P, _P, _I, _I, _I, _I, _I, _P],
    "mofa_flow_expectation_f16": [_P, _P, _I, _I, _I, _I, _F, _P],
    "mofa_filter1d_reflect_f32": [_P, _P, _P, _I, _I, _I, _I, _I, _P],
    "mofa_resize_bicubic_ac_f32": [_P, _P, _I, _I, _I, _I, _I, _P],
    "mofa_patchify_f16": [_P, _P, _I, _I, _I, _I, _I, _I, _P],
    "mofa_frames_postprocess_f32": [_P, _P, _I, _I, _I, _I, _P],
    "mofa_flow_to_image_ws_bytes": [_I, _I],
    "mofa_flow_to_image_u8": [_P, _P, _I, _I, _P, _P],
    "mofa_pose_images_f32": [_P, _P, _P, _I, _I, _I, _I, _P],
    "mofa_sparse_points_f32": [_P, _P, _I, _I, _I, _I, _I, _P, _P],
    "mofa_flow_finish_f32": [_P, _P, _P, _I, _I, _I, _I, _I, _P, _P],
}
_RESTYPE = {"mofa_softsplat_ws_bytes": C.c_int64, "mofa_flow_to_image_ws_bytes": C.c_int64}

_lib = None


class MofaHipError(RuntimeError):
    pass


def load():
    global _lib
    if _lib is not None:
        return _lib
    if not os.path.exists(LIB_PATH):
        raise MofaHipError(
            f"{LIB_PATH} not found: build it with `python -c 'import __graft_entry__ as g; g.build()'` "
            "(hipcc --offload-arch=gfx950). mofa_video_amd has no fallback path.")
    lib = C.CDLL(LIB_PATH)
    for name, argtypes in PROTOTYPES.items():
        fn = getattr(lib, name)
        fn.argtypes = argtypes
        fn.restype = _RESTYPE.get(name, C.c_int)
    _lib = lib
    return lib


def stream_ptr():
    return torch.cuda.current_stream().cuda_stream


def ptr(t):
    return None if t is None else t.data_ptr()


def check(rc, what):
    if rc != 0:
        raise MofaHipError(f"{what} failed with code {rc}")
```

mofa_video_amd/ops.py:

```python
import ctypes as C
import struct
import threading

import torch

from . import lib as L

F16 = torch.float16
F32 = torch.float32


class LaunchTimer:

    def __init__(self):
        self.rec = []
        self.tags = []

    def start(self):
        e = torch.cuda.Event(enable_timing=True)
        e.record()
        return e

    def stop(self, name, e0, flops=0.0, nbytes=0.0, tag=None):
        e1 = torch.cuda.Event(enable_timing=True)
        e1.record()
        self.rec.append((name, e0, e1, flops, nbytes))
        if tag is not None:
            self.tags.append((tag, len(self.rec) - 1))

    def by_tag(self):
        torch.cuda.synchronize()
        out = {}
        for tag, i in self.tags:
            _, e0, e1, fl, _ = self.rec[i]
            d = out.setdefault(tag, [0, 0.0, 0.0])
            d[0] += 1
            d[1] += e0.elapsed_time(e1) * 1e-3
            d[2] += fl
        return out

    def summary(self):
        torch.cuda.synchronize()
        out = {}
        for name, e0, e1, fl, nb in self.rec:
            d = out.setdefault(name, dict(launches=0, seconds=0.0, flops=0.0, bytes=0.0))
            d["launches"] += 1
            d["seconds"] += e0.elapsed_time(e1) * 1e-3
            d["flops"] += fl
            d["bytes"] += nb
        return out


TIMER = None
FORCE_TILE = L.TILE_AUTO


def _ld(t):
    assert t.dim() == 2 and t.stride(1) == 1, "token-major 2-D tensor with unit channel stride expected"
    return t.stride(0)


def _chk(t, dtype):
    assert t.is_cuda and t.dtype == dtype, f"expected cuda {dtype}, got {t.device} {t.dtype}"


class ConvGeom:
    __slots__ = ("mode", "Hin", "Win", "Hout", "Wout", "stride", "up", "T", "HW", "ksize", "dil", "pad")

    def __init__(self, mode=L.MODE_PLAIN, Hin=0, Win=0, Hout=0, Wout=0, stride=1, up=1, T=0, HW=0, ksize=3, dil=1,
                 pad=L.PAD_SAME):
        self.mode, self.Hin, self.Win, self.Hout, self.Wout = mode, Hin, Win, Hout, Wout
        self.stride, self.up, self.T, self.HW, self.ksize, self.dil, self.pad = stride, up, T, HW, ksize, dil, pad


PLAIN = ConvGeom()


def conv3x3_geom(H, W, stride=1, up=1, ksize=3, dil=1, pad=L.PAD_SAME):
    Hv, Wv = H * up, W * up
    if pad == L.PAD_TRAILING:
        span = dil * (ksize - 1) - dil * (ksize // 2)
        Ho = (Hv - 1 - span) // stride + 1
        Wo = (Wv - 1 - span) // stride + 1
    else:
        Ho = (Hv - 1) // stride + 1
        Wo = (Wv - 1) // stride + 1
    return ConvGeom(L.MODE_CONV3X3, H, W, Ho, Wo, stride, up, ksize=ksize, dil=dil, pad=pad)


def convt3_geom(T, HW):
    return ConvGeom(L.MODE_CONVT3, T=T, HW=HW)


IGEMM_WS_BYTES = 256 * 256 * 320 * 4
_igemm_ws = {}
_igemm_ws_lock = threading.Lock()


def igemm_workspace(device):
    cur = torch.cuda.current_device()
    assert device.index is None or device.index == cur, f"tensor on {device}, current device {cur}"
    key = (cur, torch.cuda.current_stream().cuda_stream)
    with _igemm_ws_lock:
        ws = _igemm_ws.pop(key, None)
        if ws is None:
            ws = torch.empty(IGEMM_WS_BYTES, dtype=torch.uint8, device=device)
            while len(_igemm_ws) >= 8:
                _igemm_ws.pop(next(iter(_igemm_ws)))
        _igemm_ws[key] = ws
    return ws


_IGEMM_ARGS = struct.Struct("@7P22i3f3iPqP")
assert _IGEMM_ARGS.size == C.sizeof(L.IgemmArgs)
_TAPS_FIXED = {L.MODE_PLAIN: 1, L.MODE_CONVT3: 3}


GN_STATS = True


def igemm(x, w, bias=None, geom=PLAIN, M=None, rowvec=None, rv=(1, 1, 1, 1 << 30), r1=None, s1=1.0, r2=None, s2=1.0,
          act=L.ACT_NONE, s_acc=1.0, out=None, tile=None, split_k=True, stats=False):
    lib = L.load()
    assert x.is_cuda and x.dtype is F16 and w.dtype is F16 and w.is_contiguous() and x.stride(1) == 1, "fp16 cuda, unit channel stride"
    N, Ktot = w.shape
    mode = geom.mode
    taps = geom.ksize * geom.ksize if mode == L.MODE_CONV3X3 else _TAPS_FIXED[mode]
    Cin = Ktot // taps
    assert Cin * taps == Ktot and x.shape[1] >= Cin, (x.shape, w.shape, taps)
    if M is None:
        if mode == L.MODE_CONV3X3:
            nimg = x.shape[0] // (geom.Hin * geom.Win)
            assert nimg * geom.Hin * geom.Win == x.shape[0]
            M = nimg * geom.Hout * geom.Wout
        else:
            M = x.shape[0]
    n_out = N // 2 if act == L.ACT_GEGLU_PAIR else N
    fresh = out is None
    if fresh:
        out = torch.empty((M, n_out), dtype=F16, device=x.device)
    else:
        assert out.dtype is F16 and out.is_cuda and out.shape[0] == M and out.shape[1] >= n_out and out.stride(1) == 1
    pb = pv = p1 = p2 = 0
    ld1 = ld2 = 0
    if bias is not None:
        assert bias.dtype is F32 and bias.numel() == N
        pb = bias.data_ptr()
    if rowvec is not None:
        assert rowvec.dtype is F32 and rowvec.dim() == 2 and rowvec.shape[1] == N and rowvec.stride(1) == 1
        assert rowvec.is_contiguous() or (rowvec.stride(0) % N == 0 and rv[1] == rowvec.stride(0) // N), (rowvec.stride(), N, rv)
        pv = rowvec.data_ptr()
    if r1 is not None:
        assert r1.dtype is F16 and r1.shape[0] == M and r1.stride(1) == 1
        p1, ld1 = r1.data_ptr(), r1.stride(0)
    if r2 is not None:
        assert r2.dtype is F16 and r2.shape[0] == M and r2.stride(1) == 1
        p2, ld2 = r2.data_ptr(), r2.stride(0)
    if split_k:
        ws = igemm_workspace(x.device)
        pw, nw = ws.data_ptr(), ws.numel()
    else:
        pw = nw = 0
    tile_ = FORCE_TILE if tile is None else tile
    st = None
    if stats and GN_STATS and fresh and M % 64 == 0 and N % 320 == 0 and act == L.ACT_NONE and r2 is None and (r1 is None or s1 == 1.0):
        st = torch.empty((M // 64, N), dtype=F32, device=x.device)
    while True:
        args = _IGEMM_ARGS.pack(x.data_ptr(), w.data_ptr(), pb, pv, p1, p2, out.data_ptr(),
                                M, N, Cin, x.stride(0), out.stride(0), ld1, ld2, mode,
                                geom.Hin, geom.Win, geom.Hout, geom.Wout, geom.stride, geom.up, geom.ksize, geom.T, geom.HW,
                                rv[0], rv[1], rv[2], rv[3], act, s_acc, s1, s2, geom.dil, geom.pad,
                                tile_, pw, nw, st.data_ptr() if st is not None else 0)
        if st is None or lib.mofa_igemm_stats_ok(args) == 1:
            break
        st = None
    t0 = TIMER.start() if TIMER is not None else None
    if split_k:
        with _igemm_ws_lock:
            rc = lib.mofa_igemm_f16(args, L.stream_ptr())
    else:
        rc = lib.mofa_igemm_f16(args, L.stream_ptr())
    if rc != 0:
        L.check(rc, "mofa_igemm_f16")
    if t0 is not None:
        TIMER.stop("igemm_f16_kernel", t0, flops=2.0 * M * N * Ktot,
                   tag=(mode, geom.stride, geom.up, M, N, Ktot, act))
    if st is not None:
        out.gn_stats = (st, _version(out), out.data_ptr())
    elif not fresh:
        _written(out)
    return out


def _version(t):
    return -1 if t.is_inference() else t._version


def _written(t):
    if t is not None and getattr(t, "gn_stats", None) is not None:
        del t.gn_stats


GN_FUSED_MAX_ENTRIES = 512


def group_norm(x, gamma, beta, nframes, HW, eps, frames_per_stat=1, silu=False, out=None, C_=None):
    lib = L.load()
    _chk(x, F16)
    Cc = C_ if C_ is not None else x.shape[1]
    assert x.shape[0] == nframes * HW
    nparts = lib.mofa_gn_nparts(HW, Cc)
    part = torch.empty((nframes, nparts, 32, 2), dtype=F32, device=x.device)
    st = L.stream_ptr()
    pairs = getattr(x, "gn_stats", None)
    if pairs is not None:
        pairs, ver, dptr = pairs
        if ver != _version(x) or dptr != x.data_ptr():
            pairs = None
    if pairs is not None and HW % 64 == 0 and Cc % 64 == 0 and tuple(pairs.shape) == (nframes * HW // 64, Cc) == (x.shape[0] // 64, x.shape[1]):
        L.check(lib.mofa_gn_partial_from_stats(L.ptr(pairs), L.ptr(part), nframes, HW, Cc, st), "mofa_gn_partial_from_stats")
        del x.gn_stats
    else:
        L.check(lib.mofa_gn_partial_f16(L.ptr(x), L.ptr(part), nframes, HW, Cc, _ld(x), st), "mofa_gn_partial_f16")
    if out is None:
        out = torch.empty((x.shape[0], Cc), dtype=F16, device=x.device)
    else:
        _written(out)
    if frames_per_stat * nparts <= GN_FUSED_MAX_ENTRIES:
        L.check(lib.mofa_gn_apply_f16(L.ptr(x), L.ptr(part), L.ptr(gamma), L.ptr(beta), L.ptr(out), nframes, HW, Cc, _ld(x),
                                      _ld(out), frames_per_stat, eps, 1 if silu else 0, st), "mofa_gn_apply_f16")
        return out
    scale = torch.empty((nframes, Cc), dtype=F32, device=x.device)
    shift = torch.empty((nframes, Cc), dtype=F32, device=x.device)
    L.check(lib.mofa_gn_finalize(L.ptr(part), L.ptr(gamma), L.ptr(beta), L.ptr(scale), L.ptr(shift), nframes, HW,
                                 Cc, frames_per_stat, eps, st), "mofa_gn_finalize")
    L.check(lib.mofa_affine_act_f16(L.ptr(x), L.ptr(scale), L.ptr(shift), L.ptr(out), nframes, HW, Cc, _ld(x), _ld(out),
                                    1 if silu else 0, st), "mofa_affine_act_f16")
    return out


def gn_nparts(HW, Cc):
    return L.load().mofa_gn_nparts(HW, Cc)


def gn_partial_into(x, part_rows, nframes, HW):
    lib = L.load()
    _chk(x, F16); _chk(part_rows, F32)
    assert x.shape[0] == nframes * HW and part_rows.is_contiguous()
    assert part_rows.shape[0] == nframes * lib.mofa_gn_nparts(HW, x.shape[1]) and part_rows.shape[1] == 64
    L.check(lib.mofa_gn_partial_f16(L.ptr(x), L.ptr(part_rows), nframes, HW, x.shape[1], _ld(x), L.stream_ptr()),
            "mofa_gn_partial_f16")


def gn_apply_gathered(x, part_all, count_per_group, gamma, beta, eps, out, nframes, HW, silu=False):
    lib = L.load()
    _chk(x, F16); _chk(out, F16); _chk(part_all, F32)
    assert x.shape[0] == nframes * HW == out.shape[0] and part_all.is_contiguous()
    _written(out)
    L.check(lib.mofa_gn_apply_gathered_f16(L.ptr(x), L.ptr(part_all), part_all.shape[0], float(count_per_group), L.ptr(gamma),
                                           L.ptr(beta), L.ptr(out), nframes, HW, x.shape[1], _ld(x), _ld(out), eps,
                                           1 if silu else 0, L.stream_ptr()), "mofa_gn_apply_gathered_f16")
    return out


def layer_norm(x, gamma, beta, eps=1e-5, rowvec=None, rv_div=1, rv_mod=1, out=None):
    lib = L.load()
    _chk(x, F16)
    M, Cc = x.shape
    if out is None:
        out = torch.empty((M, Cc), dtype=F16, device=x.device)
    else:
        _written(out)
    L.check(lib.mofa_layernorm_f16(L.ptr(x), L.ptr(gamma), L.ptr(beta), L.ptr(out), M, Cc, _ld(x), _ld(out), eps,
                                   L.ptr(rowvec), rv_div, rv_mod, L.stream_ptr()), "mofa_layernorm_f16")
    return out


_FF320_ARGS = struct.Struct("@11P7i5f4i")
assert _FF320_ARGS.size == C.sizeof(L.Ff320Args)
FF_FUSED = True


def ff320(x, w1p, b1, w2p, b2, eps=1e-5, pos=None, HW=1, T=1, r2=None, s_acc=1.0, s1=1.0, s2=0.0, out=None,
          ln_out=None, ln_eps=1e-5):
# ... 715 lines not shown
```

mofa_video_amd/weights.py:

```python
import torch

KPAD = 64


def _pad_cin(w, dim):
    cin = w.shape[dim]
    pad = (-cin) % KPAD
    if pad == 0:
        return w
    shape = list(w.shape)
    shape[dim] = pad
    return torch.cat([w, w.new_zeros(shape)], dim=dim)


def pack_linear(w):
    w = w.reshape(w.shape[0], -1)
    return _pad_cin(w, 1).to(torch.float16).contiguous()


def pack_conv3x3(w):
    w = _pad_cin(w, 1)
    n, cin, kh, kw = w.shape
    return w.permute(0, 2, 3, 1).reshape(n, kh * kw * cin).to(torch.float16).contiguous()


def pack_conv3d_t3(w):
    w = _pad_cin(w[..., 0, 0], 1)
    n, cin = w.shape[:2]
    return w.permute(0, 2, 1).reshape(n, 3 * cin).to(torch.float16).contiguous()


def pad_rows(w, mult=4):
    pad = (-w.shape[0]) % mult
    if pad == 0:
        return w
    return torch.cat([w, w.new_zeros((pad,) + tuple(w.shape[1:]))], dim=0)


def interleave_geglu(w, b):
    n2 = w.shape[0]
    ch = n2 // 2
    assert ch % 16 == 0
    idx = torch.arange(n2).reshape(2, ch // 16, 16).permute(1, 0, 2).reshape(-1)
    return w[idx].contiguous(), (b[idx].contiguous() if b is not None else None)


def pack_ff320(w1, b1, w2, gamma, beta):
    C, H = 320, 1280
    w1, w2 = w1.detach().float().cpu().reshape(2 * H, C), w2.detach().float().cpu().reshape(C, H)
    gamma, beta = gamma.detach().float().cpu(), beta.detach().float().cpu()
    b1f = (b1.detach().float().cpu() if b1 is not None else torch.zeros(2 * H)) + w1 @ beta
    w1g = (w1 * gamma[None, :]).to(torch.float16)
    lane = torch.arange(64)
    n, lh = lane % 32, lane // 32
    c, t, s_, e = torch.arange(40), torch.arange(2), torch.arange(20), torch.arange(8)
    rows = (t[None, :, None, None, None] * H + 32 * c[:, None, None, None, None] + n[None, None, None, :, None])
    cols = 16 * s_[None, None, :, None, None] + 8 * lh[None, None, None, :, None] + e[None, None, None, None, :]
    w1p = w1g[rows.expand(40, 2, 20, 64, 8), cols.expand(40, 2, 20, 64, 8)].contiguous()
    j, u, jj = torch.arange(10), torch.arange(2), torch.arange(8)
    rows2 = 32 * j[None, :, None, None, None] + n[None, None, None, :, None]
    cols2 = (32 * c[:, None, None, None, None] + 16 * u[None, None, :, None, None] + 4 * lh[None, None, None, :, None] +
             (jj & 3)[None, None, None, None, :] + 8 * (jj >> 2)[None, None, None, None, :])
    w2p = w2.to(torch.float16)[rows2.expand(40, 10, 2, 64, 8), cols2.expand(40, 10, 2, 64, 8)].contiguous()
    return w1p, b1f.contiguous(), w2p


def pack_lin320(w, b=None, gamma=None, beta=None):
    w = w.detach().float().cpu().reshape(w.shape[0], -1)
    N, K = w.shape
    assert K == 320 and N % 64 == 0, (N, K)
    bias = b.detach().float().cpu().clone() if b is not None else None
    if beta is not None:
        bias = (bias if bias is not None else torch.zeros(N)) + w @ beta.detach().float().cpu()
    if gamma is not None:
        w = w * gamma.detach().float().cpu()[None, :]
    wh = w.to(torch.float16)
    lane = torch.arange(64)
    n, lh = lane % 32, lane // 32
    c, t, s_, e = torch.arange(N // 64), torch.arange(2), torch.arange(20), torch.arange(8)
    rows = 64 * c[:, None, None, None, None] + 32 * t[None, :, None, None, None] + n[None, None, None, :, None]
    cols = 16 * s_[None, None, :, None, None] + 8 * lh[None, None, None, :, None] + e[None, None, None, None, :]
    shp = (N // 64, 2, 20, 64, 8)
    return wh[rows.expand(shp), cols.expand(shp)].contiguous(), (bias.contiguous() if bias is not None else None)


def f32(t):
    return t.detach().to(torch.float32).contiguous()
```

Before: 4.211 frames/s.

## Fold nearest-upsample-by-2 into 3x3 conv as four 2x2 phase convolutions

Adds a new igemm mode that folds a 2x nearest upsample followed by a 3x3 conv into four output phases, each a 2x2 conv on the low-resolution input with pre-summed weights. This cuts the reduction from 9 taps to 4 per output pixel for the upsampler convs in the UNet decoder and VAE. The tile kernels (256x256 and 256x320) gain an UP2F cursor, phase-dependent weight offsets and a scattered output-row epilogue, and the split-K fixup handles the same remapping. Weights are folded in fp32 and then rounded to fp16, so numerics shift slightly. The path is gated by an environment flag and a plan check.

```diff
diff --git a/include/mofa_hip.h b/include/mofa_hip.h
--- a/include/mofa_hip.h
+++ b/include/mofa_hip.h
@@ -15,7 +15,8 @@
 
 int mofa_version(void);
 
-enum { MOFA_MODE_PLAIN = 0, MOFA_MODE_CONV3X3 = 1, MOFA_MODE_CONVT3 = 2 };
+enum { MOFA_MODE_PLAIN = 0, MOFA_MODE_CONV3X3 = 1, MOFA_MODE_CONVT3 = 2,
+       MOFA_MODE_CONV3X3_UP2F = 3 };
 enum { MOFA_ACT_NONE = 0, MOFA_ACT_SILU = 1, MOFA_ACT_GEGLU_PAIR = 2, MOFA_ACT_RELU = 3,
        MOFA_ACT_GELU = 4  };
 
@@ -58,6 +59,7 @@
     int32_t reserved[4];
 } mofa_igemm_plan_t;
 int mofa_igemm_plan(const mofa_igemm_args* a, int n_cu, mofa_igemm_plan_t* out);
+int64_t mofa_igemm_up2f_row(const mofa_igemm_args* a, int64_t tile_row);
 
 int mofa_attn_spatial_f16(const void* q, const void* k, const void* v, void* out,
                           int nframes, int heads, int head_dim, int S, int ldq, int ldk, int ldv, int ldo, float scale,
diff --git a/mofa_video_amd/blocks.py b/mofa_video_amd/blocks.py
--- a/mofa_video_amd/blocks.py
+++ b/mofa_video_amd/blocks.py
@@ -4,7 +4,7 @@
 
 from . import lib as L
 from . import ops
-from .weights import (f32, interleave_geglu, pack_conv3d_t3, pack_conv3x3, pack_ff320, pack_lin320, pack_linear, pad_rows)
+from .weights import (f32, fold_up2, interleave_geglu, pack_conv3d_t3, pack_conv3x3, pack_ff320, pack_lin320, pack_linear, pad_rows)
 
 BIG = 1 << 30
 LOCAL_STREAM_ABOVE = 128
@@ -94,8 +94,28 @@
         self.w = s.dev(pack_conv3x3(w))
         self.b = s.dev(f32(b))
         self.stride, self.up, self.pad = stride, up, pad
+        self.wf = s.dev(fold_up2(w)) if up == 2 and stride == 1 and pad == L.PAD_SAME else None
+        self._fold = {}
+
+    def _folded(self, x, H, W, kw):
+        if self.wf is None or not ops.UP2_FOLD or not x.is_cuda:
+            return False
+        if not set(kw) <= {"out", "split_k", "act", "stats", "tile"}:
+            return False
+        if kw.get("act", L.ACT_NONE) != L.ACT_NONE or kw.get("stats") or kw.get("tile") is not None:
+            return False
+        out = kw.get("out")
+        key = (H, W, x.shape[0], ops.FORCE_TILE, x.stride(0), x.data_ptr() & 15,
+               None if out is None else (out.stride(0), out.data_ptr() & 15))
+        ok = self._fold.get(key)
+        if ok is None:
+            ok = self._fold[key] = ops.igemm_up2f_ok(x, self.wf, self.b, H, W, out)
+        return ok
 
     def __call__(self, x, H, W, **kw):
+        if self._folded(x, H, W, kw):
+            kw = {k: v for k, v in kw.items() if k in ("out", "split_k")}
+            return ops.igemm(x, self.wf, self.b, geom=ops.conv3x3_up2f_geom(H, W), **kw)
         return ops.igemm(x, self.w, self.b, geom=ops.conv3x3_geom(H, W, self.stride, self.up, pad=self.pad), **kw)
 
 
diff --git a/mofa_video_amd/csrc/igemm.hip b/mofa_video_amd/csrc/igemm.hip
--- a/mofa_video_amd/csrc/igemm.hip
+++ b/mofa_video_amd/csrc/igemm.hip
@@ -417,6 +417,12 @@
 
 extern "C" int mofa_igemm_stats_ok(const mofa_igemm_args* a) { return igemm320_stats_ok(a) ? 1 : 0; }
 
+extern "C" int64_t mofa_igemm_up2f_row(const mofa_igemm_args* a, int64_t tile_row) {
+    if (igemm_check_args(a) != MOFA_OK || a->mode != MOFA_MODE_CONV3X3_UP2F) return MOFA_EINVAL;
+    if (tile_row < 0 || tile_row >= 256ll * igemm_tiles_m(a, 256)) return MOFA_EINVAL;
+    return igemm_up2f_out_row(*a, (int)tile_row);
+}
+
 extern "C" int mofa_igemm_plan(const mofa_igemm_args* a, int n_cu, mofa_igemm_plan_t* out) {
     if (!a || !out || n_cu <= 0) return MOFA_EINVAL;
     *out = igemm_plan(a, n_cu);
diff --git a/mofa_video_amd/csrc/igemm320.hip b/mofa_video_amd/csrc/igemm320.hip
--- a/mofa_video_amd/csrc/igemm320.hip
+++ b/mofa_video_amd/csrc/igemm320.hip
@@ -29,10 +29,11 @@
     unsigned wo0;
 };
 
-template <int EPI, bool SPLIT = false, bool STATS = false>
+template <int EPI, bool SPLIT = false, bool STATS = false, bool UP2F = false>
 __global__ __launch_bounds__(512, 2) void igemm320_f16_kernel(const mofa_igemm_args a, const int tilesN, const int ntiles,
                                                               const Aux aux) {
     constexpr bool R1 = (EPI & EPI_R1) != 0, R2 = (EPI & EPI_R2) != 0, RV = (EPI & EPI_RV) != 0, GEGLU = (EPI & EPI_GEGLU) != 0;
+    typedef typename SelectT<UP2F, CursorUp2f<::Cursor3>, ::Cursor3>::type Cursor3;
     extern __shared__ __attribute__((aligned(16))) char smem[];
     TileWalk walk;
     walk.init(ntiles);
@@ -44,7 +45,7 @@
     const int wm = wave / WN3, wn = wave - wm * WN3;
     const int l31 = lane & 31, lh = lane >> 5;
 
-    const int taps = igemm_taps(a);
+    const int taps = kernel_taps<UP2F>(a);
     const int kpt = a.Cin / 64, nk = taps * kpt;
     const size_t Ktot = (size_t)taps * a.Cin;
 
@@ -79,27 +80,47 @@
         item_decode(c.phase, c.local, tile, kb, ke);
         const int tm = fdiv(tile, aux.tiles_n), tn = tile - tm * tilesN;
         const int l = lane_now(lane), r_l = l >> 2;
-        const int g0 = pack_geo(a, aux, tm * TBM3 + 16 * wave + r_l), g1 = pack_geo(a, aux, tm * TBM3 + 16 * (wave + 8) + r_l);
-        c.gx0 = live ? g0 : -1;
-        c.gx1 = live ? g1 : -1;
-        const unsigned wo = (unsigned)(tn * TBN3 + 16 * wave + r_l) * (unsigned)(Ktot * 2) + swz_bytes(l, p);
-        c.wo0 = live ? wo : W_DEAD;
+        if constexpr (UP2F) {
+            const int g0 = pack_geo_up2f(a, aux, tm * TBM3 + 16 * wave + r_l), g1 = pack_geo_up2f(a, aux, tm * TBM3 + 16 * (wave + 8) + r_l);
+            c.gx0 = live ? g0 : -1;
+            c.gx1 = live ? g1 : -1;
+            c.ph = tm & 3;
+            const unsigned wo = (unsigned)(c.ph * a.N + tn * TBN3 + 16 * wave + r_l) * (unsigned)(Ktot * 2) + swz_bytes(l, p);
+            c.wo0 = live ? wo : W_DEAD;
+        } else {
+            const int g0 = pack_geo(a, aux, tm * TBM3 + 16 * wave + r_l), g1 = pack_geo(a, aux, tm * TBM3 + 16 * (wave + 8) + r_l);
+            c.gx0 = live ? g0 : -1;
+            c.gx1 = live ? g1 : -1;
+            const unsigned wo = (unsigned)(tn * TBN3 + 16 * wave + r_l) * (unsigned)(Ktot * 2) + swz_bytes(l, p);
+            c.wo0 = live ? wo : W_DEAD;
+        }
         c.ikc = 0; c.ksw = 0; c.ky = 0; c.kx = 0;
         c.kend = ke;
         if constexpr (SPLIT) {
             int tap = fdiv(kb, aux.kpt_d);
             c.ikc = kb - tap * kpt;
             c.ksw = kb;
-            if (a.mode == MOFA_MODE_CONV3X3) { c.ky = fdiv(tap, aux.ks_d); c.kx = tap - c.ky * tg.ks; } else c.ky = tap;
-            c.xo0 = tap_src(a, aux, tg, c.gx0, c.ky, c.kx, swz_bytes(l, p));
-            c.xo1 = tap_src(a, aux, tg, c.gx1, c.ky, c.kx, swz_bytes(l, p));
+            if constexpr (UP2F) {
+                c.ky = tap >> 1; c.kx = tap & 1;
+                c.xo0 = tap_src_up2f(a, aux, c.gx0, c.ky, c.kx, c.ph, swz_bytes(l, p));
+                c.xo1 = tap_src_up2f(a, aux, c.gx1, c.ky, c.kx, c.ph, swz_bytes(l, p));
+            } else {
+                if (a.mode == MOFA_MODE_CONV3X3) { c.ky = fdiv(tap, aux.ks_d); c.kx = tap - c.ky * tg.ks; } else c.ky = tap;
+                c.xo0 = tap_src(a, aux, tg, c.gx0, c.ky, c.kx, swz_bytes(l, p));
+                c.xo1 = tap_src(a, aux, tg, c.gx1, c.ky, c.kx, swz_bytes(l, p));
+            }
         }
     };
     auto issue = [&](Cursor3& c, const int p, const int slot) __attribute__((always_inline)) {
         if (c.ikc == 0) {
             const int l = lane_now(lane);
-            c.xo0 = tap_src(a, aux, tg, c.gx0, c.ky, c.kx, swz_bytes(l, p));
-            c.xo1 = tap_src(a, aux, tg, c.gx1, c.ky, c.kx, swz_bytes(l, p));
+            if constexpr (UP2F) {
+                c.xo0 = tap_src_up2f(a, aux, c.gx0, c.ky, c.kx, c.ph, swz_bytes(l, p));
+                c.xo1 = tap_src_up2f(a, aux, c.gx1, c.ky, c.kx, c.ph, swz_bytes(l, p));
+            } else {
+                c.xo0 = tap_src(a, aux, tg, c.gx0, c.ky, c.kx, swz_bytes(l, p));
+                c.xo1 = tap_src(a, aux, tg, c.gx1, c.ky, c.kx, swz_bytes(l, p));
+            }
         }
         char* pl = smem + slot + p * PLANE;
         const int wk = c.ksw * 128;
@@ -110,7 +131,7 @@
         if (grp == p) bglds16(rsw, c.wo0 + wd2, wk, pl + XPL + (16 + (wave & 3)) * 1024);
     };
     auto advance = [&](Cursor3& c, const int p) __attribute__((always_inline)) {
-        tap_advance(c, a, kpt, tg.ks);
+        if constexpr (UP2F) tap_advance_up2f(c, kpt); else tap_advance(c, a, kpt, tg.ks);
         if (c.ksw == c.kend) { next_pos(c.phase, c.local); cur_setup(c, p); }
     };
 
@@ -234,7 +255,12 @@
                 for (int p = 0; p < 4; ++p) {
                     const H16Piece r = h16_row<8>(eb, srow, lane, p);
                     const int mr = mw + 32 * i + r.row, n = nw + 32 * j0 + 8 * r.blk;
-                    if (mr < a.M && n + 8 <= a.N) *(f16x8*)(out + (size_t)mr * a.ldo + n) = r.v;
+                    if constexpr (UP2F) {
+                        const int orow = up2f_out_row(a, aux, mr);
+                        if (orow >= 0 && n + 8 <= a.N) *(f16x8*)(out + (size_t)orow * a.ldo + n) = r.v;
+                    } else if (mr < a.M && n + 8 <= a.N) {
+                        *(f16x8*)(out + (size_t)mr * a.ldo + n) = r.v;
+                    }
                 }
             }
             {
@@ -250,7 +276,12 @@
                 for (int p = 0; p < 2; ++p) {
                     const H16Piece r = h16_row<4>(eb, srow, lane, p);
                     const int mr = mw + 32 * i + r.row, n = nw + 32 * JS + 8 * r.blk;
-                    if (mr < a.M && n + 8 <= a.N) *(f16x8*)(out + (size_t)mr * a.ldo + n) = r.v;
+                    if constexpr (UP2F) {
+                        const int orow = up2f_out_row(a, aux, mr);
+                        if (orow >= 0 && n + 8 <= a.N) *(f16x8*)(out + (size_t)orow * a.ldo + n) = r.v;
+                    } else if (mr < a.M && n + 8 <= a.N) {
+                        *(f16x8*)(out + (size_t)mr * a.ldo + n) = r.v;
+                    }
                 }
             }
         }
@@ -690,6 +721,9 @@
                     else epilogue_res16(IC<1>{}, IC<0>{}, acc, mw, nw, eb);
                 }
             }
+        } else if constexpr (UP2F) {
+            if (wn == 0) epilogue_light(IC<MOFA_ACT_NONE>{}, IC<0>{}, acc, mw, nw, eb);
+            else epilogue_light(IC<MOFA_ACT_NONE>{}, IC<1>{}, acc, mw, nw, eb);
         } else if (RV && idx_u < 0) {
             epilogue_rows(IC<0>{}, acc, mw, nw, eb);
         } else if (wn == 0) {
@@ -709,6 +743,7 @@
 
 typedef void (*igemm320_kern_t)(const mofa_igemm_args, const int, const int, const Aux);
 
+template <bool UP2F = false>
 __global__ __launch_bounds__(256) void igemm320_fixup_kernel(const mofa_igemm_args a, const float* __restrict__ ws, const int tile0,
                                                              const int nsplit, const int tilesN, const int R) {
     constexpr int PPR = TBN3 / 8, PPT = TBM3 * PPR;
@@ -717,8 +752,14 @@
         const int r = (int)(idx / PPT), rem = (int)(idx - (long long)r * PPT);
         const int rr = rem / PPR, pc = rem - rr * PPR;
         const int tile = tile0 + r, tm = tile / tilesN, tn = tile - tm * tilesN;
-        const int m = tm * TBM3 + rr, n = tn * TBN3 + pc * 8;
-        if (m >= a.M || n + 8 > a.N) continue;
+        int m = tm * TBM3 + rr;
+        const int n = tn * TBN3 + pc * 8;
+        if constexpr (UP2F) {
+            m = igemm_up2f_out_row(a, m);
+            if (m < 0 || n + 8 > a.N) continue;
+        } else if (m >= a.M || n + 8 > a.N) {
+            continue;
+        }
         float v[8];
 #pragma unroll
         for (int e = 0; e < 8; ++e) v[e] = 0.f;
@@ -791,6 +832,7 @@
 static const igemm320_kern_t k_igemm320[9] = {igemm320_f16_kernel<0>, igemm320_f16_kernel<1>, igemm320_f16_kernel<2>,
                                                igemm320_f16_kernel<3>, igemm320_f16_kernel<4>, igemm320_f16_kernel<5>,
                                                igemm320_f16_kernel<6>, nullptr, igemm320_f16_kernel<8>};
+static const igemm320_kern_t k_igemm320_up2f[2] = {igemm320_f16_kernel<0, false, false, true>, igemm320_f16_kernel<0, true, false, true>};
 static const igemm320_kern_t k_igemm320_split[7] = {
     igemm320_f16_kernel<0, true>, igemm320_f16_kernel<1, true>, igemm320_f16_kernel<2, true>, igemm320_f16_kernel<3, true>,
     igemm320_f16_kernel<4, true>, igemm320_f16_kernel<5, true>, igemm320_f16_kernel<6, true>};
@@ -802,6 +844,7 @@
 
 int igemm320_init() {
     return mofa_lds_optin(k_igemm320, LDS_BYTES3) == MOFA_OK && mofa_lds_optin(k_igemm320_split, LDS_BYTES3) == MOFA_OK &&
+                   mofa_lds_optin(k_igemm320_up2f, LDS_BYTES3) == MOFA_OK &&
                    mofa_lds_optin(k_igemm320_stats, LDS_BYTES3) == MOFA_OK && mofa_lds_optin(k_igemm320_split_stats, LDS_BYTES3) == MOFA_OK
                ? MOFA_OK
                : MOFA_ELAUNCH;
@@ -811,9 +854,10 @@
 int igemm320_launch(const mofa_igemm_args* a, const IgemmPlan& plan, hipStream_t stream) {
     const int kind = plan.kind, S = plan.split, R = plan.rem_tiles, tilesN = plan.tiles_n;
     Aux aux = igemm_pipe_aux(a, igemm_taps(*a), tilesN);
-    igemm320_kern_t kern = a->stats ? k_igemm320_stats[kind] : k_igemm320[kind];
+    const bool up2f = a->mode == MOFA_MODE_CONV3X3_UP2F;
+    igemm320_kern_t kern = up2f ? k_igemm320_up2f[0] : a->stats ? k_igemm320_stats[kind] : k_igemm320[kind];
     if (S > 1) {
-        kern = a->stats ? k_igemm320_split_stats[kind] : k_igemm320_split[kind];
+        kern = up2f ? k_igemm320_up2f[1] : a->stats ? k_igemm320_split_stats[kind] : k_igemm320_split[kind];
         aux.nsplit = S, aux.nsplit_d = fastdiv_make(S);
         aux.tile0 = plan.full_tiles, aux.nitems = R * S, aux.ws = (float*)a->workspace;
     }
@@ -821,7 +865,11 @@
     MOFA_CHECK_LAUNCH();
     if (S == 1) return MOFA_OK;
     const long long pieces = (long long)R * TBM3 * (TBN3 / 8);
-    hipLaunchKernelGGL(igemm320_fixup_kernel, dim3((int)((pieces + 255) / 256)), dim3(256), 0, stream, *a,
+    if (up2f)
+        hipLaunchKernelGGL(igemm320_fixup_kernel<true>, dim3((int)((pieces + 255) / 256)), dim3(256), 0, stream, *a,
+                           (const float*)a->workspace, plan.full_tiles, S, tilesN, R);
+    else
+        hipLaunchKernelGGL(igemm320_fixup_kernel<false>, dim3((int)((pieces + 255) / 256)), dim3(256), 0, stream, *a,
                        (const float*)a->workspace, plan.full_tiles, S, tilesN, R);
     MOFA_CHECK_LAUNCH();
     if (a->stats) {
diff --git a/mofa_video_amd/csrc/igemm8.hip b/mofa_video_amd/csrc/igemm8.hip
--- a/mofa_video_amd/csrc/igemm8.hip
+++ b/mofa_video_amd/csrc/igemm8.hip
@@ -19,11 +19,12 @@
     unsigned wo0, wo1, wo2, wo3;
 };
 
-template <int EPI, int VAR = 0>
+template <int EPI, int VAR = 0, bool UP2F = false>
 __global__ __launch_bounds__(512, 2) void igemm8_f16_kernel(const mofa_igemm_args a, const int tilesN, const int ntiles,
                                                             const Aux aux) {
     constexpr bool GEGLU = (EPI & EPI_GEGLU) != 0, R1 = (EPI & EPI_R1) != 0, R2 = (EPI & EPI_R2) != 0,
                    RV = (EPI & EPI_RV) != 0;
+    typedef typename SelectT<UP2F, CursorUp2f<::Cursor>, ::Cursor>::type Cursor;
     extern __shared__ __attribute__((aligned(16))) char smem[];
     TileWalk walk;
     walk.init(ntiles);
@@ -34,7 +35,7 @@
     const int wm = wave / WN, wn = wave - wm * WN;
     const int l31 = lane & 31, lh = lane >> 5;
 
-    const int taps = igemm_taps(a);
+    const int taps = kernel_taps<UP2F>(a);
     const int kpt = a.Cin / BKS, nk = taps * kpt;
     const size_t Ktot = (size_t)taps * a.Cin;
 
@@ -49,13 +50,20 @@
         const int tile = walk.start + (live ? c.local : 0);
         const int tm = fdiv(tile, aux.tiles_n), tn = tile - tm * tilesN;
         const int l = lane_now(lane), hr_l = 16 * wave + (l >> 3);
-        const int g0 = pack_geo(a, aux, tm * TBM + x_row(h, 0, hr_l)), g1 = pack_geo(a, aux, tm * TBM + x_row(h, 1, hr_l));
+        int g0, g1;
+        if constexpr (UP2F) {
+            g0 = pack_geo_up2f(a, aux, tm * TBM + x_row(h, 0, hr_l)), g1 = pack_geo_up2f(a, aux, tm * TBM + x_row(h, 1, hr_l));
+            c.ph = tm & 3;
+        } else {
+            g0 = pack_geo(a, aux, tm * TBM + x_row(h, 0, hr_l)), g1 = pack_geo(a, aux, tm * TBM + x_row(h, 1, hr_l));
+        }
         c.gx0 = live ? g0 : -1;
         c.gx1 = live ? g1 : -1;
         if (with_w) {
             auto w_off = [&](int hq) __attribute__((always_inline)) {
                 int n = tn * TBN + w_row(hq >> 1, hq & 1, hr_l);
                 n = n < a.N ? n : a.N - 1;
+                if constexpr (UP2F) n += c.ph * a.N;
                 const unsigned o = (unsigned)n * (unsigned)(Ktot * 2) + swz_bytes(l, hq & 1);
                 return live ? o : XO_INVALID;
             };
@@ -66,8 +74,13 @@
     auto issue_x = [&](Cursor& c, const int h, const int bo) __attribute__((always_inline)) {
         if (c.ikc == 0) {
             const int l = lane_now(lane);
-            c.xo0 = tap_src(a, aux, tg, c.gx0, c.ky, c.kx, swz_bytes(l, 0));
-            c.xo1 = tap_src(a, aux, tg, c.gx1, c.ky, c.kx, swz_bytes(l, 1));
+            if constexpr (UP2F) {
+                c.xo0 = tap_src_up2f(a, aux, c.gx0, c.ky, c.kx, c.ph, swz_bytes(l, 0));
+                c.xo1 = tap_src_up2f(a, aux, c.gx1, c.ky, c.kx, c.ph, swz_bytes(l, 1));
+            } else {
+                c.xo0 = tap_src(a, aux, tg, c.gx0, c.ky, c.kx, swz_bytes(l, 0));
+                c.xo1 = tap_src(a, aux, tg, c.gx1, c.ky, c.kx, swz_bytes(l, 1));
+            }
         }
         bglds16(rsx, c.xo0, c.ikc * (BKS * 2), smem + bo + x_row(h, 0, 16 * wave) * RB);
         bglds16(rsx, c.xo1, c.ikc * (BKS * 2), smem + bo + x_row(h, 1, 16 * wave) * RB);
@@ -79,7 +92,7 @@
         bglds16(rsw, c.wo3, c.ksw * (BKS * 2), smem + bo + SXB + w_row(1, 1, 16 * wave) * RB);
     };
     auto advance = [&](Cursor& c, const int h, const bool with_w) __attribute__((always_inline)) {
-        tap_advance(c, a, kpt, tg.ks);
+        if constexpr (UP2F) tap_advance_up2f(c, kpt); else tap_advance(c, a, kpt, tg.ks);
         if (c.ksw == nk) { c.local += walk.stride; cur_setup(c, h, with_w); }
     };
 
@@ -265,7 +278,12 @@
                 for (int p = 0; p < 4; ++p) {
                     const H16Piece r = h16_row<4 * NJ>(scr, RowLines128{}, lane, p);
                     const int mr = mw + 32 * i + r.row, n = nw + 8 * r.blk;
-                    if (mr < a.M && n + 8 <= nout) *(f16x8*)(out + (size_t)mr * a.ldo + n) = r.v;
+                    if constexpr (UP2F) {
+                        const int orow = up2f_out_row(a, aux, mr);
+                        if (orow >= 0 && n + 8 <= nout) *(f16x8*)(out + (size_t)orow * a.ldo + n) = r.v;
+                    } else if (mr < a.M && n + 8 <= nout) {
+                        *(f16x8*)(out + (size_t)mr * a.ldo + n) = r.v;
+                    }
                 }
             }
         }
@@ -418,6 +436,8 @@
         } else if constexpr (RV) {
             if (idx_u >= 0) epilogue_light(IC<MOFA_ACT_NONE>{}, IC<1>{}, acc, mw, nw, idx_u);
             else epilogue_light(IC<MOFA_ACT_NONE>{}, IC<0>{}, acc, mw, nw, 0);
+        } else if constexpr (UP2F) {
+            epilogue_light(IC<MOFA_ACT_NONE>{}, IC<0>{}, acc, mw, nw, 0);
         } else {
             if (a.act == MOFA_ACT_NONE) epilogue_light(IC<MOFA_ACT_NONE>{}, IC<0>{}, acc, mw, nw, 0);
             else if (a.act == MOFA_ACT_SILU) epilogue_light(IC<MOFA_ACT_SILU>{}, IC<0>{}, acc, mw, nw, 0);
@@ -440,7 +460,7 @@
 static const igemm8_kern_t k_igemm8[9] = {igemm8_f16_kernel<0>, igemm8_f16_kernel<1>, igemm8_f16_kernel<2>,
                                            igemm8_f16_kernel<3>, igemm8_f16_kernel<4>, igemm8_f16_kernel<5>,
                                            igemm8_f16_kernel<6>, igemm8_f16_kernel<7>, igemm8_f16_kernel<8>};
-
+static const igemm8_kern_t k_igemm8_up2f[1] = {igemm8_f16_kernel<0, 0, true>};
 
 #ifdef MOFA_PROBE
 static int s_probe_var = 0;
@@ -459,7 +479,7 @@
 #endif
 
 int igemm8_init() {
-    if (mofa_lds_optin(k_igemm8, LDS_BYTES) != MOFA_OK) return MOFA_ELAUNCH;
+    if (mofa_lds_optin(k_igemm8, LDS_BYTES) != MOFA_OK || mofa_lds_optin(k_igemm8_up2f, LDS_BYTES) != MOFA_OK) return MOFA_ELAUNCH;
 #ifdef MOFA_PROBE
     if (mofa_lds_optin(k_probe_kern, LDS_BYTES) != MOFA_OK || mofa_lds_optin(k_trace_kern, LDS_BYTES) != MOFA_OK) return MOFA_ELAUNCH;
 #endif
@@ -470,7 +490,7 @@
     static_assert(TBM == 256 && TBN == 256 && LDS_BYTES == 163840, "igemm_plan.h's MOFA_TILE_256X256 row");
     const int kind = plan.kind;
     Aux aux = igemm_pipe_aux(a, igemm_taps(*a), plan.tiles_n);
-    igemm8_kern_t kern = k_igemm8[kind];
+    igemm8_kern_t kern = a->mode == MOFA_MODE_CONV3X3_UP2F ? k_igemm8_up2f[0] : k_igemm8[kind];
 #ifdef MOFA_PROBE
     aux.trace = s_probe_trace;
     if (kind == 0 && s_probe_var)
diff --git a/mofa_video_amd/csrc/igemm_pipe.h b/mofa_video_amd/csrc/igemm_pipe.h
--- a/mofa_video_amd/csrc/igemm_pipe.h
+++ b/mofa_video_amd/csrc/igemm_pipe.h
@@ -65,6 +65,38 @@
     return ok ? off : XO_INVALID;
 }
 
+template <bool UP2F>
+__device__ __forceinline__ int kernel_taps(const mofa_igemm_args& a) {
+    if constexpr (UP2F) return 4; else return igemm_taps_classic(a);
+}
+template <bool B, class T, class F> struct SelectT { typedef T type; };
+template <class T, class F> struct SelectT<false, T, F> { typedef F type; };
+template <class C> struct CursorUp2f : C { int ph; };
+struct FDivBy { FastDiv d; __device__ __forceinline__ int operator()(int n) const { return fdiv(n, d); } };
+__device__ __forceinline__ int pack_geo_up2f(const mofa_igemm_args& a, const Aux& aux, int m) {
+    const IgemmUp2fPixel s = igemm_up2f_pixel(a, m, FDivBy{aux.hw}, FDivBy{aux.wout});
+    const int g = (s.img << 20) | (s.y << 10) | s.x;
+    return s.valid ? g : -1;
+}
+__device__ __forceinline__ unsigned tap_src_up2f(const mofa_igemm_args& a, const Aux& aux, int g, int ky, int kx, int ph, int swzb) {
+    const int vy = ((g >> 10) & 1023) + ky - (1 - (ph >> 1)), vx = (g & 1023) + kx - (1 - (ph & 1));
+    const bool ok = g >= 0 && vy >= 0 && vx >= 0 && vy < a.Hin && vx < a.Win;
+    const int row = ((g >> 20) * a.Hin + vy) * a.Win + vx;
+    const unsigned off = (unsigned)row * (unsigned)aux.ldxb + (unsigned)swzb;
+    return ok ? off : XO_INVALID;
+}
+template <class C>
+__device__ __forceinline__ void tap_advance_up2f(C& c, const int kpt) {
+    ++c.ksw;
+    if (++c.ikc == kpt) {
+        c.ikc = 0;
+        if (++c.kx == 2) { c.kx = 0; ++c.ky; }
+    }
+}
+__device__ __forceinline__ int up2f_out_row(const mofa_igemm_args& a, const Aux& aux, int mr) {
+    return igemm_up2f_out_row(a, mr, FDivBy{aux.hw}, FDivBy{aux.wout});
+}
+
 template <class C>
 __device__ __forceinline__ void tap_advance(C& c, const mofa_igemm_args& a, const int kpt, const int ks) {
     ++c.ksw;
@@ -147,8 +179,9 @@
 static inline Aux igemm_pipe_aux(const mofa_igemm_args* a, int taps, int tilesN) {
     Aux aux;
     aux.tiles_n = fastdiv_make(tilesN);
-    aux.hw = fastdiv_make(a->mode == MOFA_MODE_CONV3X3 ? a->Hout * a->Wout : 1);
-    aux.wout = fastdiv_make(a->mode == MOFA_MODE_CONV3X3 ? a->Wout : 1);
+    const bool up2f = a->mode == MOFA_MODE_CONV3X3_UP2F;
+    aux.hw = fastdiv_make(up2f ? a->Hin * a->Win : a->mode == MOFA_MODE_CONV3X3 ? a->Hout * a->Wout : 1);
+    aux.wout = fastdiv_make(up2f ? a->Win : a->mode == MOFA_MODE_CONV3X3 ? a->Wout : 1);
     aux.t3hw = fastdiv_make(a->mode == MOFA_MODE_CONVT3 ? a->HW : 1);
     aux.t3t = fastdiv_make(a->mode == MOFA_MODE_CONVT3 && a->T > 0 ? a->T : 1);
     const bool halo = a->mode == MOFA_MODE_CONVT3 && a->T == 0;
@@ -156,7 +189,7 @@
     aux.row_shift = halo ? a->HW : 0;
     aux.xbase = (const char*)a->x - (halo ? (size_t)a->HW * a->ldx * 2 : 0);
     aux.x_bytes = (unsigned)(igemm8_rows_in(a) * a->ldx * 2 - (a->ldx - a->Cin) * 2);
-    aux.w_bytes = (unsigned)((long long)a->N * taps * a->Cin * 2);
+    aux.w_bytes = (unsigned)(igemm_w_rows(a) * taps * a->Cin * 2);
     aux.trace = nullptr;
     aux.nsplit_d = fastdiv_make(1);
     aux.kpt_d = fastdiv_make(a->Cin / 64);
diff --git a/mofa_video_amd/csrc/igemm_plan.h b/mofa_video_amd/csrc/igemm_plan.h
--- a/mofa_video_amd/csrc/igemm_plan.h
+++ b/mofa_video_amd/csrc/igemm_plan.h
@@ -17,8 +17,34 @@
 
 static inline int igemm_cdiv(int64_t a, int64_t b) { return (int)((a + b - 1) / b); }
 
+__attribute__((always_inline)) constexpr int igemm_taps_classic(const mofa_igemm_args& a) {
+    return (a.mode == MOFA_MODE_CONV3X3) ? (a.ksize > 0 ? a.ksize * a.ksize : 9) : (a.mode == MOFA_MODE_CONVT3 ? 3 : 1);
+}
 __attribute__((always_inline)) constexpr int igemm_taps(const mofa_igemm_args& a) {
-    return (a.mode == MOFA_MODE_CONV3X3) ? (a.ksize > 0 ? a.ksize * a.ksize : 9) : (a.mode == MOFA_MODE_CONVT3 ? 3 : 1);
+    return a.mode == MOFA_MODE_CONV3X3_UP2F ? 4 : igemm_taps_classic(a);
+}
+
+static inline long long igemm_w_rows(const mofa_igemm_args* a) { return a->mode == MOFA_MODE_CONV3X3_UP2F ? 4ll * a->N : a->N; }
+static inline int igemm_tiles_m(const mofa_igemm_args* a, int tm) {
+    return a->mode == MOFA_MODE_CONV3X3_UP2F ? 4 * (int)((a->M / 4 + 255) / 256) : (int)(((long long)a->M + tm - 1) / tm);
+}
+struct IgemmUp2fPixel { int ph, img, y, x, valid; };
+template <class DivHW, class DivW>
+__attribute__((always_inline)) constexpr IgemmUp2fPixel igemm_up2f_pixel(const mofa_igemm_args& a, int r, DivHW div_hw, DivW div_w) {
+    const int q = ((r >> 10) << 8) | (r & 255);
+    const int img = div_hw(q), rem = q - img * (a.Hin * a.Win);
+    const int y = div_w(rem);
+    return IgemmUp2fPixel{(r >> 8) & 3, img, y, rem - y * a.Win, q < (a.M >> 2) ? 1 : 0};
+}
+template <class DivHW, class DivW>
+__attribute__((always_inline)) constexpr int igemm_up2f_out_row(const mofa_igemm_args& a, int r, DivHW div_hw, DivW div_w) {
+    const IgemmUp2fPixel s = igemm_up2f_pixel(a, r, div_hw, div_w);
+    const int o = (s.img * a.Hout + 2 * s.y + (s.ph >> 1)) * a.Wout + 2 * s.x + (s.ph & 1);
+    return s.valid ? o : -1;
+}
+struct IgemmPlainDiv { int d; constexpr int operator()(int n) const { return n / d; } };
+constexpr int igemm_up2f_out_row(const mofa_igemm_args& a, int r) {
+    return igemm_up2f_out_row(a, r, IgemmPlainDiv{a.Hin * a.Win}, IgemmPlainDiv{a.Win});
 }
 
 static inline int igemm_grid(long long ntiles, int slots) {
@@ -27,7 +53,7 @@
 }
 
 static inline long long igemm8_rows_in(const mofa_igemm_args* a) {
-    if (a->mode == MOFA_MODE_CONV3X3) return a->M / ((long long)a->Hout * a->Wout) * a->Hin * a->Win;
+    if (a->mode == MOFA_MODE_CONV3X3 || a->mode == MOFA_MODE_CONV3X3_UP2F) return a->M / ((long long)a->Hout * a->Wout) * a->Hin * a->Win;
     if (a->mode == MOFA_MODE_CONVT3 && a->T == 0) return (long long)a->M + 2ll * a->HW;
     return a->M;
 }
@@ -40,8 +66,10 @@
     if (a->bias && (((uintptr_t)a->bias) & 15)) return false;
     if ((a->r1 || a->r2 || a->rowvec) && a->act != MOFA_ACT_NONE) return false;
     if (a->rowvec && (((uintptr_t)a->rowvec) & 15)) return false;
-    if ((long long)a->N * Ktot * 2 >= (1ll << 32) || (((uintptr_t)a->w) & 15)) return false;
-    if (a->mode == MOFA_MODE_CONV3X3) {
+    if (igemm_w_rows(a) * Ktot * 2 >= (1ll << 32) || (((uintptr_t)a->w) & 15)) return false;
+    if (a->mode == MOFA_MODE_CONV3X3_UP2F) {
+        if (a->M > 0x7fff0000) return false;
+    } else if (a->mode == MOFA_MODE_CONV3X3) {
         const long long nimg = a->M / ((long long)a->Hout * a->Wout);
         if (a->Hout > 1024 || a->Wout > 1024 || nimg > 2047) return false;
     } else if (a->mode == MOFA_MODE_CONVT3) {
@@ -53,7 +81,7 @@
 
 static inline bool igemm320_eligible(const mofa_igemm_args* a, int kind, int taps) {
     if (kind == 7 || !igemm_pipe_eligible(a, kind, (long long)taps * a->Cin)) return false;
-    return (long long)(a->N + 320) * taps * a->Cin * 2 < 0x7ff00000LL;
+    return (igemm_w_rows(a) + 320) * taps * a->Cin * 2 < 0x7ff00000LL;
 }
 
 static inline bool igemm320_stats_ok(const mofa_igemm_args* a) {
@@ -82,7 +110,7 @@
     if (!a || !a->x || !a->w || !a->out) return MOFA_EINVAL;
     if (a->M <= 0 || a->N <= 0 || a->Cin <= 0) return MOFA_EINVAL;
     if (a->Cin % 64 != 0 || a->N % 4 != 0) return MOFA_EINVAL;
-    if (a->mode < 0 || a->mode > 2 || a->act < 0 || a->act > MOFA_ACT_GELU) return MOFA_EINVAL;
+    if (a->mode < 0 || a->mode > MOFA_MODE_CONV3X3_UP2F || a->act < 0 || a->act > MOFA_ACT_GELU) return MOFA_EINVAL;
     if (a->mode == MOFA_MODE_CONV3X3) {
         if (a->Hin <= 0 || a->Win <= 0 || a->Hout <= 0 || a->Wout <= 0) return MOFA_EINVAL;
         if ((a->stride != 1 && a->stride != 2) || (a->up != 1 && a->up != 2)) return MOFA_EINVAL;
@@ -90,6 +118,15 @@
         if (a->dil < 0 || (a->dil > 1 && a->up != 1)) return MOFA_EINVAL;
         if (a->pad != MOFA_PAD_SAME && a->pad != MOFA_PAD_TRAILING) return MOFA_EINVAL;
         if (a->M % (a->Hout * a->Wout) != 0 || a->Hout > 65535 || a->Wout > 65535) return MOFA_EINVAL;
+    }
+    if (a->mode == MOFA_MODE_CONV3X3_UP2F) {
+        if (a->Hin <= 0 || a->Win <= 0 || a->Hin > 1024 || a->Win > 1024) return MOFA_EINVAL;
+        if (a->Hout != 2 * a->Hin || a->Wout != 2 * a->Win || a->stride != 1 || a->up != 2) return MOFA_EINVAL;
+        if ((a->ksize != 0 && a->ksize != 3) || (a->dil != 0 && a->dil != 1) || a->pad != MOFA_PAD_SAME) return MOFA_EINVAL;
+        if (a->M % (a->Hout * a->Wout) != 0 || a->M / (a->Hout * a->Wout) > 2047) return MOFA_EINVAL;
+        if (a->act != MOFA_ACT_NONE || a->r1 || a->r2 || a->rowvec || a->stats) return MOFA_EINVAL;
+        if (a->tile == MOFA_TILE_128X128 || a->tile == MOFA_TILE_192X128) return MOFA_EINVAL;
+        if (!igemm_pipe_eligible(a, 0, 4ll * a->Cin)) return MOFA_EINVAL;
     }
     if (a->mode == MOFA_MODE_CONVT3 && (a->T < 0 || a->HW <= 0 || (a->T > 0 && a->M % (a->T * a->HW) != 0)))
         return MOFA_EINVAL;
@@ -112,7 +149,7 @@
     const double nk = (double)(Ktot / 64);
     int choice = 0;
     double best = 0;
-    for (int k = 0; k < 2; ++k) {
+    for (int k = 0; k < 2 && a->mode != MOFA_MODE_CONV3X3_UP2F; ++k) {
         const IgemmTile& c = igemm_tile(ids[k]);
         const long long t = (long long)igemm_cdiv(a->M, c.tm) * igemm_cdiv(a->N, c.tn);
         const long long slots_k = (long long)n_cu * c.wg_per_cu;
@@ -120,13 +157,13 @@
         if (choice == 0 || cost < best) { best = cost; choice = ids[k]; }
     }
     {
-        const long long t = (long long)igemm_cdiv(a->M, 256) * igemm_cdiv(a->N, 256);
+        const long long t = (long long)igemm_tiles_m(a, 256) * igemm_cdiv(a->N, 256);
         const double cost = (double)((t + n_cu - 1) / n_cu) * 256 * 256 * 0.62 * (1.0 + epi8[kind] / nk);
-        if (cost < best) { best = cost; choice = MOFA_TILE_256X256; }
+        if (choice == 0 || cost < best) { best = cost; choice = MOFA_TILE_256X256; }
     }
     if (kind != 7) {
         static const double epi320[9] = {3.0, 7.5, 8.5, 9.5, 3.5, 7.9, 9.0, 12.0, 5.0};
-        const long long t = (long long)igemm_cdiv(a->M, 256) * igemm_cdiv(a->N, 320);
+        const long long t = (long long)igemm_tiles_m(a, 256) * igemm_cdiv(a->N, 320);
         const int S = kind == 8 ? 1 : igemm320_split(t, (int)nk, n_cu, a->workspace ? a->workspace_bytes : 0);
         const double rounds = S > 1 ? (double)(t / n_cu) + 1.0 / S + 0.12 : (double)((t + n_cu - 1) / n_cu);
         const int tn320 = igemm_cdiv(a->N, 320);
@@ -153,8 +190,9 @@
         if (forced) return refused;
         choice = chain[i + 1];
     }
+    if (a->mode == MOFA_MODE_CONV3X3_UP2F && choice != MOFA_TILE_256X320 && choice != MOFA_TILE_256X256) return refused;
     const IgemmTile& c = igemm_tile(choice);
-    const int tilesM = igemm_cdiv(a->M, c.tm), tilesN = igemm_cdiv(a->N, c.tn);
+    const int tilesM = igemm_tiles_m(a, c.tm), tilesN = igemm_cdiv(a->N, c.tn);
     const long long nt = (long long)tilesM * tilesN;
     if (nt > 0x7fffffffLL) return refused;
     if (a->stats && (((uintptr_t)a->stats) & 15)) return refused;
diff --git a/mofa_video_amd/lib.py b/mofa_video_amd/lib.py
--- a/mofa_video_amd/lib.py
+++ b/mofa_video_amd/lib.py
@@ -6,7 +6,7 @@
 _HERE = os.path.dirname(os.path.abspath(__file__))
 LIB_PATH = os.environ.get("MOFA_HIP_LIB") or os.path.join(_HERE, "libmofa_hip.so")
 
-MODE_PLAIN, MODE_CONV3X3, MODE_CONVT3 = 0, 1, 2
+MODE_PLAIN, MODE_CONV3X3, MODE_CONVT3, MODE_CONV3X3_UP2F = 0, 1, 2, 3
 ACT_NONE, ACT_SILU, ACT_GEGLU_PAIR, ACT_RELU, ACT_GELU = 0, 1, 2, 3, 4
 PAD_SAME, PAD_TRAILING = 0, 1
 SPARSE_ADD, SPARSE_LAST = 0, 1
@@ -84,6 +84,7 @@
     "mofa_igemm_f16": [_P, _P],
     "mofa_igemm_stats_ok": [_P],
     "mofa_igemm_plan": [_P, _I, _P],
+    "mofa_igemm_up2f_row": [_P, _L],
     "mofa_ff320_f16": [_P, _P],
     "mofa_lin320_f16": [_P, _P],
     "mofa_attn_spatial_f16": [_P, _P, _P, _P, _I, _I, _I, _I, _I, _I, _I, _I, _F, _P],
@@ -150,7 +151,7 @@
     "mofa_sparse_points_f32": [_P, _P, _I, _I, _I, _I, _I, _P, _P],
     "mofa_flow_finish_f32": [_P, _P, _P, _I, _I, _I, _I, _I, _P, _P],
 }
-_RESTYPE = {"mofa_softsplat_ws_bytes": C.c_int64, "mofa_flow_to_image_ws_bytes": C.c_int64}
+_RESTYPE = {"mofa_igemm_up2f_row": C.c_int64, "mofa_softsplat_ws_bytes": C.c_int64, "mofa_flow_to_image_ws_bytes": C.c_int64}
 
 _lib = None
 
diff --git a/mofa_video_amd/ops.py b/mofa_video_amd/ops.py
--- a/mofa_video_amd/ops.py
+++ b/mofa_video_amd/ops.py
@@ -1,4 +1,5 @@
 import ctypes as C
+import os
 import struct
 import threading
 
@@ -86,6 +87,10 @@
         Ho = (Hv - 1) // stride + 1
         Wo = (Wv - 1) // stride + 1
     return ConvGeom(L.MODE_CONV3X3, H, W, Ho, Wo, stride, up, ksize=ksize, dil=dil, pad=pad)
+
+
+def conv3x3_up2f_geom(H, W):
+    return ConvGeom(L.MODE_CONV3X3_UP2F, H, W, 2 * H, 2 * W, 1, 2, ksize=3, dil=1, pad=L.PAD_SAME)
 
 
 def convt3_geom(T, HW):
@@ -113,7 +118,25 @@
 
 _IGEMM_ARGS = struct.Struct("@7P22i3f3iPqP")
 assert _IGEMM_ARGS.size == C.sizeof(L.IgemmArgs)
-_TAPS_FIXED = {L.MODE_PLAIN: 1, L.MODE_CONVT3: 3}
+_TAPS_FIXED = {L.MODE_PLAIN: 1, L.MODE_CONVT3: 3, L.MODE_CONV3X3_UP2F: 4}
+
+UP2_FOLD = os.environ.get("MOFA_UP2_FOLD", "1") != "0"
+
+
+def igemm_up2f_ok(x, wf, bias, H, W, out=None):
+    lib = L.load()
+    nimg = x.shape[0] // (H * W)
+    if not x.is_cuda or nimg * H * W != x.shape[0]:
+        return False
+    N, Cin = wf.shape[0] // 4, wf.shape[1] // 4
+    args = _IGEMM_ARGS.pack(x.data_ptr(), wf.data_ptr(), bias.data_ptr() if bias is not None else 0, 0, 0, 0,
+                            out.data_ptr() if out is not None else 256,
+                            nimg * 4 * H * W, N, Cin, x.stride(0), out.stride(0) if out is not None else N, 0, 0, L.MODE_CONV3X3_UP2F,
+                            H, W, 2 * H, 2 * W, 1, 2, 3, 0, 0, 1, 1, 1, 1 << 30, L.ACT_NONE, 1.0, 1.0, 1.0, 1, L.PAD_SAME,
+                            FORCE_TILE, 256, IGEMM_WS_BYTES, 0)
+    plan = L.IgemmPlan()
+    n_cu = torch.cuda.get_device_properties(x.device).multi_processor_count
+    return lib.mofa_igemm_plan(args, n_cu, C.byref(plan)) == 0 and plan.rc == 0
 
 
 GN_STATS = True
@@ -125,11 +148,14 @@
     assert x.is_cuda and x.dtype is F16 and w.dtype is F16 and w.is_contiguous() and x.stride(1) == 1, "fp16 cuda, unit channel stride"
     N, Ktot = w.shape
     mode = geom.mode
+    if mode == L.MODE_CONV3X3_UP2F:
+        assert N % 4 == 0
+        N //= 4
     taps = geom.ksize * geom.ksize if mode == L.MODE_CONV3X3 else _TAPS_FIXED[mode]
     Cin = Ktot // taps
     assert Cin * taps == Ktot and x.shape[1] >= Cin, (x.shape, w.shape, taps)
     if M is None:
-        if mode == L.MODE_CONV3X3:
+        if mode in (L.MODE_CONV3X3, L.MODE_CONV3X3_UP2F):
             nimg = x.shape[0] // (geom.Hin * geom.Win)
             assert nimg * geom.Hin * geom.Win == x.shape[0]
             M = nimg * geom.Hout * geom.Wout
diff --git a/mofa_video_amd/weights.py b/mofa_video_amd/weights.py
--- a/mofa_video_amd/weights.py
+++ b/mofa_video_amd/weights.py
@@ -22,6 +22,15 @@
     w = _pad_cin(w, 1)
     n, cin, kh, kw = w.shape
     return w.permute(0, 2, 3, 1).reshape(n, kh * kw * cin).to(torch.float16).contiguous()
+
+
+def fold_up2(w):
+    w = _pad_cin(w, 1).to(torch.float16).to(torch.float32)
+    n, cin, kh, kw = w.shape
+    assert kh == 3 and kw == 3, w.shape
+    sel = torch.tensor([[[1., 0., 0.], [0., 1., 1.]], [[1., 1., 0.], [0., 0., 1.]]], device=w.device)
+    f = torch.einsum("ayk,bxl,nckl->abnyxc", sel, sel, w)
+    return f.reshape(4 * n, 4 * cin).to(torch.float16).contiguous()
 
 
 def pack_conv3d_t3(w):
```

New measurement: 4.272 frames/s (median of 6 runs). +1.4%, better.
